# claudiok/clsim

Measured on AMD Instinct MI355X. Metric: propagated photons/sec (whole node), higher is better.
Workload: dtype f32

## Files before the change

### clsim_amd/_lib.py

```python
import ctypes as C
import os

HERE = os.path.dirname(os.path.abspath(__file__))
LIB_PATH = os.environ.get("CLSIMHIP_LIB", os.path.join(HERE, "libclsimhip.so"))

OK, ERR_ARGUMENT, ERR_STATE, ERR_CONFIG, ERR_DEVICE, ERR_IO = 0, -1, -2, -3, -4, -5
REFINDEX_ICECUBE, REFINDEX_TABLE, REFINDEX_DISPERSION = 0, 1, 2

DP = C.POINTER(C.c_double)


class Function(C.Structure):
    _fields_ = [("kind", C.c_int32), ("n", C.c_int32), ("start", C.c_double), ("step", C.c_double),
                ("values", DP), ("value", C.c_double), ("wavelengths", DP)]


class RandomValue(C.Structure):
    _fields_ = [("kind", C.c_int32), ("n", C.c_int32), ("first", C.c_double), ("spacing", C.c_double),
                ("y", DP), ("value", C.c_double), ("x", DP)]


class StepRequest(C.Structure):
    _fields_ = [("x", C.c_float), ("y", C.c_float), ("z", C.c_float), ("time", C.c_float),
                ("dx", C.c_float), ("dy", C.c_float), ("dz", C.c_float), ("length", C.c_float),
                ("pa", C.c_float), ("pb", C.c_float), ("kind", C.c_uint32), ("identifier", C.c_uint32),
                ("photons_per_step", C.c_uint32), ("num_photons_in_last_step", C.c_uint32), ("num_steps", C.c_uint64)]


class PPCConfig(C.Structure):
    _fields_ = [("photons_per_step", C.c_uint32), ("high_photons_per_step", C.c_uint32), ("use_high_photons_per_step_from", C.c_double),
                ("use_cascade_extension", C.c_int32), ("reserved", C.c_int32), ("medium_density", C.c_double), ("seed", C.c_uint64)]


class Distribution(C.Structure):
    _fields_ = [("kind", C.c_int32), ("value", C.c_float)]


class FlasherConfig(C.Structure):
    _fields_ = [("polar", Distribution), ("azimuthal", Distribution), ("time_delay", Distribution),
                ("interpret_in_polar_coordinates", C.c_int32), ("photons_per_step", C.c_uint32),
                ("max_bunch_size", C.c_uint32), ("bunch_size_granularity", C.c_uint32)]


class Axis(C.Structure):
    _fields_ = [("kind", C.c_int32), ("min", C.c_double), ("max", C.c_double), ("n_bins", C.c_uint32), ("power", C.c_uint32)]


class Polynomial(C.Structure):
    _fields_ = [("n", C.c_int32), ("coefficients", DP), ("range_min", C.c_double), ("range_max", C.c_double),
                ("underflow", C.c_double), ("overflow", C.c_double)]


class MediumDesc(C.Structure):
    _fields_ = [("num_layers", C.c_int32), ("layers_z_start", C.c_double), ("layers_height", C.c_double),
                ("min_wavelength", C.c_double), ("max_wavelength", C.c_double),
                ("lengths_kind", C.c_int32), ("abs_length", DP), ("sca_length", DP),
                ("alpha", C.c_double), ("kappa", C.c_double), ("A", C.c_double), ("B", C.c_double),
                ("D", C.c_double), ("E", C.c_double),
                ("a_dust400", DP), ("delta_tau", DP), ("b400", DP),
                ("n", C.c_double * 5), ("g", C.c_double * 5),
                ("scatter_kind", C.c_int32), ("liu_fraction", C.c_double), ("mean_cosine", C.c_double),
                ("has_anisotropy", C.c_int32), ("aniso_azimuth", C.c_double), ("aniso_k1", C.c_double),
                ("aniso_k2", C.c_double),
                ("has_pre_transform", C.c_int32), ("pre_renormalize", C.c_int32), ("pre_matrix", C.c_double * 9),
                ("has_post_transform", C.c_int32), ("post_renormalize", C.c_int32), ("post_matrix", C.c_double * 9),
                ("has_tilt", C.c_int32), ("tilt_num_distances", C.c_int32), ("tilt_num_z", C.c_int32),
                ("tilt_distances", DP), ("tilt_z_coordinates", DP), ("tilt_z_corrections", DP),
                ("tilt_azimuth", C.c_double),
                ("table_num_wavelengths", C.c_int32), ("table_start_wavelength", C.c_double),
                ("table_wavelength_step", C.c_double), ("table_store_as_16bit", C.c_int32),
                ("abs_length_table", DP), ("sca_length_table", DP),
                ("phase_index_kind", C.c_int32), ("group_index_kind", C.c_int32),
                ("phase_index_table", Function), ("group_index_table", Function)]


SYMBOLS = [
    "clsimhip_medium_create", "clsimhip_medium_create_from_ppc",
    "clsimhip_medium_create_from_photonics", "clsimhip_medium_describe", "clsimhip_medium_destroy",
    "clsimhip_icecube_dom_acceptance", "clsimhip_make_cherenkov_wlen_generator", "clsimhip_make_wlen_generator",
    "clsimhip_mwc_multipliers", "clsimhip_mwc_multipliers_from_file", "clsimhip_seed_streams",
    "clsimhip_create", "clsimhip_destroy", "clsimhip_last_error", "clsimhip_set_device", "clsimhip_get_device", "clsimhip_uses_pooled_kernel", "clsimhip_kernel_for_bunch",
    "clsimhip_step_series_blob_size", "clsimhip_encode_step_series", "clsimhip_decode_step_series",
    "clsimhip_photon_series_blob_size", "clsimhip_encode_photon_series", "clsimhip_decode_photon_series", "clsimhip_encode_portable_uint",
    "clsimhip_comm_get_unique_id", "clsimhip_comm_create", "clsimhip_comm_destroy", "clsimhip_gather_hits",
    "clsimhip_comm_info", "clsimhip_comm_statistics",
    "clsimhip_set_wlen_generators", "clsimhip_set_wlen_bias", "clsimhip_set_medium_properties", "clsimhip_set_geometry",
    "clsimhip_set_geometry_from_text_file",
    "clsimhip_set_enable_double_buffering", "clsimhip_set_double_precision", "clsimhip_set_stop_detected_photons",
    "clsimhip_set_save_all_photons", "clsimhip_set_save_all_photons_prescale",
    "clsimhip_set_fixed_number_of_absorption_lengths", "clsimhip_set_dom_pancake_factor",
    "clsimhip_set_photon_history_entries", "clsimhip_set_workgroup_size", "clsimhip_set_max_num_workitems",
    "clsimhip_compile", "clsimhip_get_max_workgroup_size", "clsimhip_initialize", "clsimhip_initialize_with_streams",
    "clsimhip_is_initialized", "clsimhip_enqueue_steps", "clsimhip_get_conversion_result", "clsimhip_get_result_histories",
    "clsimhip_release_result",
    "clsimhip_get_workgroup_size", "clsimhip_get_max_num_workitems", "clsimhip_queue_size",
    "clsimhip_more_photons_available", "clsimhip_get_statistics", "clsimhip_propagate_device",
    "clsimhip_set_concurrent_device_launches",
    "clsimhip_replace_indices_with_ids", "clsimhip_kernel_time_ms", "clsimhip_get_table", "clsimhip_get_rng_state",
    "clsimhip_eval_math", "clsimhip_check_math_exhaustive", "clsimhip_version",
    "clsimhip_eval_device_function", "clsimhip_eval_device_random", "clsimhip_get_option",
    "clsimhip_set_tuning", "clsimhip_get_tuning", "clsimhip_tabulator_set_tuning",
    "clsimhip_get_last_launch", "clsimhip_tabulator_get_last_launch",
    "clsimhip_count_generated_steps", "clsimhip_generate_steps_device", "clsimhip_generate_steps",
    "clsimhip_ppc_create", "clsimhip_ppc_destroy", "clsimhip_ppc_photons_per_meter", "clsimhip_ppc_enqueue", "clsimhip_shower_parameters",
    "clsimhip_flasher_correction_factor", "clsimhip_flasher_enqueue",
    "clsimhip_feeder_create", "clsimhip_feeder_destroy", "clsimhip_feeder_enqueue_light_source", "clsimhip_feeder_enqueue_steps",
    "clsimhip_feeder_enqueue_barrier", "clsimhip_feeder_barrier_active", "clsimhip_feeder_more_steps_available",
    "clsimhip_feeder_get_conversion_result", "clsimhip_feeder_release_result",
    "clsimhip_count_flasher_steps", "clsimhip_generate_flasher_steps_device", "clsimhip_generate_flasher_steps",
    "clsimhip_flasher_time_profile",
    "clsimhip_step_store_create", "clsimhip_step_store_destroy", "clsimhip_step_store_insert", "clsimhip_step_store_size",
    "clsimhip_step_store_count", "clsimhip_step_store_pop_bunch", "clsimhip_step_store_pop_bunch_filled",
    "clsimhip_step_store_size_with_dummy_fill",
    "clsimhip_tabulator_create", "clsimhip_tabulator_destroy", "clsimhip_tabulator_last_error",
    "clsimhip_tabulator_enqueue_steps", "clsimhip_tabulator_finish", "clsimhip_tabulator_get_shape",
    "clsimhip_tabulator_get_bin_content", "clsimhip_tabulator_get_bin_sums", "clsimhip_tabulator_get_bin_edges",
    "clsimhip_tabulator_get_statistics", "clsimhip_tabulator_get_rng_state", "clsimhip_tabulator_get_table",
    "clsimhip_tabulator_write_fits_file",
    "clsimhip_mcpe_generator_create", "clsimhip_mcpe_generator_destroy", "clsimhip_mcpe_generator_last_error",
    "clsimhip_mcpe_convert_host", "clsimhip_mcpe_convert_device", "clsimhip_set_mcpe_generator", "clsimhip_get_result_mcpes",
    "clsimhip_mcpe_series_host", "clsimhip_mcpe_series_workspace_bytes", "clsimhip_mcpe_series_device", "clsimhip_set_mcpe_series",
    "clsimhip_enqueue_steps_with_particles", "clsimhip_get_result_mcpe_series",
    "clsimhip_mcpe_merge_host", "clsimhip_mcpe_merge_workspace_bytes", "clsimhip_mcpe_merge_device", "clsimhip_set_mcpe_merging",
    "clsimhip_get_result_mcpe_merged",
    "clsimhip_pmt_generator_create", "clsimhip_pmt_generator_destroy", "clsimhip_pmt_generator_last_error",
    "clsimhip_pmt_convert_host", "clsimhip_pmt_convert_device", "clsimhip_set_pmt_generator", "clsimhip_get_result_pmt_hits",
]

KERNEL_FAMILIES = ("classic", "keep", "pool", "pool_keep", "tab4", "tab5")
LENGTHS_KINDS = ("constant", "icecube", "table")


def launched_dict(out):
    v = [int(x) for x in out]
    if v[0] < 0:
        return None
    return dict(family=KERNEL_FAMILIES[v[0]], lengths=LENGTHS_KINDS[v[1]], tilt=bool(v[2]), aniso=bool(v[3]), flasher=bool(v[4]), fast=bool(v[5]))


_lib = None


def load():
    global _lib
    if _lib is not None:
        return _lib
    if not os.path.exists(LIB_PATH):
        raise ImportError("%s is missing: run `python -c 'import __graft_entry__ as g; g.build()'` "
                          "(make -C clsim_amd/csrc); the HIP propagator has no fallback path" % LIB_PATH)
    try:
        import torch
    except ImportError:
        pass
    lib = C.CDLL(LIB_PATH)
    vp, sz, u32, u64, i32, dbl = C.c_void_p, C.c_size_t, C.c_uint32, C.c_uint64, C.c_int, C.c_double
    sig = {
        "clsimhip_medium_create": (i32, [C.POINTER(MediumDesc), C.POINTER(vp)]),
        "clsimhip_medium_create_from_ppc": (i32, [C.c_char_p, dbl, i32, C.POINTER(vp)]),
        "clsimhip_medium_create_from_photonics": (i32, [C.c_char_p, dbl, C.POINTER(vp)]),
        "clsimhip_medium_describe": (i32, [vp, C.POINTER(MediumDesc)]),
        "clsimhip_medium_destroy": (None, [vp]),
        "clsimhip_icecube_dom_acceptance": (i32, [dbl, dbl, DP, DP, DP]),
        "clsimhip_make_cherenkov_wlen_generator": (i32, [C.POINTER(Function), vp, DP, DP, DP]),
        "clsimhip_make_wlen_generator": (i32, [C.POINTER(Function), C.POINTER(Function), vp, C.POINTER(RandomValue), DP, DP, C.c_size_t]),
        "clsimhip_mwc_multipliers": (i32, [vp, sz]),
        "clsimhip_mwc_multipliers_from_file": (i32, [C.c_char_p, vp, sz]),
        "clsimhip_seed_streams": (i32, [vp, sz, u64, vp]),
        "clsimhip_create": (i32, [i32, C.POINTER(vp)]),
        "clsimhip_destroy": (None, [vp]),
        "clsimhip_last_error": (C.c_char_p, [vp]),
        "clsimhip_set_device": (i32, [vp, i32]),
        "clsimhip_get_device": (i32, [vp, C.POINTER(i32)]),
        "clsimhip_uses_pooled_kernel": (i32, [vp, C.POINTER(i32)]),
        "clsimhip_kernel_for_bunch": (i32, [vp, sz, C.POINTER(i32)]),
        "clsimhip_step_series_blob_size": (i32, [sz, C.POINTER(sz)]),
        "clsimhip_encode_step_series": (i32, [vp, sz, vp, sz, C.POINTER(sz)]),
        "clsimhip_decode_step_series": (i32, [vp, sz, vp, sz, C.POINTER(sz), C.POINTER(sz)]),
        "clsimhip_photon_series_blob_size": (i32, [sz, C.POINTER(sz)]),
        "clsimhip_encode_photon_series": (i32, [vp, sz, vp, sz, C.POINTER(sz)]),
        "clsimhip_decode_photon_series": (i32, [vp, sz, vp, sz, C.POINTER(sz), C.POINTER(sz)]),
        "clsimhip_encode_portable_uint": (i32, [u64, vp, C.POINTER(sz)]),
        "clsimhip_comm_get_unique_id": (i32, [vp]),
        "clsimhip_comm_create": (i32, [i32, i32, i32, vp, C.POINTER(vp)]),
        "clsimhip_comm_destroy": (None, [vp]),
        "clsimhip_comm_info": (i32, [vp, vp, vp, vp, vp, C.c_size_t]),
        "clsimhip_comm_statistics": (i32, [vp, vp, vp, vp, vp, i32]),
        "clsimhip_gather_hits": (i32, [vp, vp, vp, sz, i32, vp, sz, vp, vp]),
        "clsimhip_set_wlen_generators": (i32, [vp, C.POINTER(RandomValue), sz]),
        "clsimhip_set_wlen_bias": (i32, [vp, C.POINTER(Function)]),
        "clsimhip_set_medium_properties": (i32, [vp, vp]),
        "clsimhip_set_geometry": (i32, [vp, sz, vp, vp, vp, vp, vp, C.POINTER(C.c_char_p), dbl]),
        "clsimhip_set_geometry_from_text_file": (i32, [vp, C.c_char_p, dbl, C.c_int32, C.c_int32, u32, u32]),
        "clsimhip_set_enable_double_buffering": (i32, [vp, i32]),
        "clsimhip_set_double_precision": (i32, [vp, i32]),
        "clsimhip_set_stop_detected_photons": (i32, [vp, i32]),
        "clsimhip_set_save_all_photons": (i32, [vp, i32]),
        "clsimhip_set_save_all_photons_prescale": (i32, [vp, dbl]),
        "clsimhip_set_fixed_number_of_absorption_lengths": (i32, [vp, dbl]),
        "clsimhip_set_dom_pancake_factor": (i32, [vp, dbl]),
        "clsimhip_set_photon_history_entries": (i32, [vp, u32]),
        "clsimhip_set_workgroup_size": (i32, [vp, sz]),
        "clsimhip_set_max_num_workitems": (i32, [vp, sz]),
        "clsimhip_compile": (i32, [vp]),
        "clsimhip_get_max_workgroup_size": (i32, [vp, C.POINTER(sz)]),
        "clsimhip_initialize": (i32, [vp, u64]),
        "clsimhip_initialize_with_streams": (i32, [vp, vp, vp, sz]),
        "clsimhip_is_initialized": (i32, [vp]),
        "clsimhip_enqueue_steps": (i32, [vp, vp, sz, u32]),
        "clsimhip_get_conversion_result": (i32, [vp, C.POINTER(u32), C.POINTER(vp), C.POINTER(sz)]),
        "clsimhip_get_result_histories": (i32, [vp, vp, C.POINTER(C.POINTER(C.c_float)), C.POINTER(u32)]),
        "clsimhip_release_result": (i32, [vp, vp]),
        "clsimhip_get_workgroup_size": (i32, [vp, C.POINTER(sz)]),
        "clsimhip_get_max_num_workitems": (i32, [vp, C.POINTER(sz)]),
        "clsimhip_queue_size": (i32, [vp, C.POINTER(sz)]),
        "clsimhip_more_photons_available": (i32, [vp, C.POINTER(i32)]),
        "clsimhip_get_statistics": (i32, [vp, DP]),
        "clsimhip_propagate_device": (i32, [vp, vp, sz, sz, vp, sz, vp, vp]),
        "clsimhip_set_concurrent_device_launches": (i32, [vp, i32]),
        "clsimhip_replace_indices_with_ids": (i32, [vp, vp, sz]),
        "clsimhip_kernel_time_ms": (i32, [vp, i32, DP, C.POINTER(u64)]),
        "clsimhip_get_table": (C.c_long, [vp, C.c_char_p, DP, sz]),
        "clsimhip_get_rng_state": (i32, [vp, vp, sz]),
        "clsimhip_eval_math": (i32, [i32, i32, vp, vp, sz, vp]),
        "clsimhip_get_option": (i32, [vp, i32, DP]),
        "clsimhip_set_tuning": (i32, [vp, C.c_char_p, C.c_longlong]),
        "clsimhip_get_tuning": (i32, [vp, C.c_char_p, C.POINTER(C.c_longlong)]),
        "clsimhip_tabulator_set_tuning": (i32, [vp, C.c_char_p, C.c_longlong]),
        "clsimhip_get_last_launch": (i32, [vp, C.POINTER(C.c_int)]),
        "clsimhip_tabulator_get_last_launch": (i32, [vp, C.POINTER(C.c_int)]),
        "clsimhip_eval_device_function": (i32, [vp, i32, i32, i32, vp, sz, vp]),
        "clsimhip_eval_device_random": (i32, [vp, i32, i32, i32, vp, vp, sz, sz, vp]),
        "clsimhip_check_math_exhaustive": (i32, [i32, i32, i32, i32, vp, sz]),
        "clsimhip_version": (C.c_char_p, []),
        "clsimhip_ppc_create": (i32, [vp, C.POINTER(Function), C.POINTER(PPCConfig), C.POINTER(vp)]),
        "clsimhip_ppc_destroy": (None, [vp]),
        "clsimhip_ppc_photons_per_meter": (i32, [vp, i32, C.POINTER(C.c_double)]),
        "clsimhip_ppc_enqueue": (i32, [vp, vp, sz, C.POINTER(StepRequest), sz, C.POINTER(sz)]),
        "clsimhip_shower_parameters": (i32, [i32, C.c_double, C.c_double, C.POINTER(C.c_double)]),
        "clsimhip_flasher_correction_factor": (i32, [C.POINTER(Function), C.c_double, C.POINTER(Function), C.c_double, C.c_double, C.POINTER(C.c_double)]),
        "clsimhip_flasher_enqueue": (i32, [C.c_double, u64, vp, sz, vp, sz, C.POINTER(sz)]),
        "clsimhip_feeder_create": (i32, [vp, i32, u64, sz, sz, sz, C.POINTER(vp)]),
        "clsimhip_feeder_destroy": (None, [vp]),
        "clsimhip_feeder_enqueue_light_source": (i32, [vp, vp]),
        "clsimhip_feeder_enqueue_steps": (i32, [vp, u32, vp, sz]),
        "clsimhip_feeder_enqueue_barrier": (i32, [vp]),
        "clsimhip_feeder_barrier_active": (i32, [vp, C.POINTER(C.c_int)]),
        "clsimhip_feeder_more_steps_available": (i32, [vp, C.POINTER(C.c_int)]),
        "clsimhip_feeder_get_conversion_result": (i32, [vp, C.c_double, C.POINTER(C.c_int), C.POINTER(vp), C.POINTER(sz), C.POINTER(vp), C.POINTER(sz), C.POINTER(C.c_int)]),
        "clsimhip_feeder_release_result": (i32, [vp, vp]),
        "clsimhip_count_generated_steps": (i32, [C.POINTER(StepRequest), sz, sz, C.POINTER(sz), C.POINTER(sz)]),
        "clsimhip_generate_steps_device": (i32, [i32, C.POINTER(StepRequest), sz, u64, sz, vp, sz, vp, C.POINTER(sz)]),
        "clsimhip_generate_steps": (i32, [i32, C.POINTER(StepRequest), sz, u64, sz, vp, sz, C.POINTER(sz)]),
        "clsimhip_count_flasher_steps": (i32, [C.POINTER(FlasherConfig), vp, sz, C.POINTER(sz), C.POINTER(sz)]),
        "clsimhip_generate_flasher_steps_device": (i32, [i32, C.POINTER(FlasherConfig), vp, sz, u64, vp, sz, vp, C.POINTER(sz)]),
        "clsimhip_generate_flasher_steps": (i32, [i32, C.POINTER(FlasherConfig), vp, sz, u64, vp, sz, C.POINTER(sz)]),
        "clsimhip_flasher_time_profile": (i32, [dbl, vp, vp]),
        "clsimhip_step_store_create": (i32, [sz, C.POINTER(vp)]),
        "clsimhip_step_store_destroy": (None, [vp]),
        "clsimhip_step_store_insert": (i32, [vp, vp, sz]),
        "clsimhip_step_store_size": (i32, [vp, C.POINTER(sz)]),
        "clsimhip_step_store_count": (i32, [vp, u32, C.POINTER(u32)]),
        "clsimhip_step_store_pop_bunch": (i32, [vp, sz, vp, C.POINTER(sz)]),
        "clsimhip_step_store_pop_bunch_filled": (i32, [vp, sz, vp, vp]),
        "clsimhip_step_store_size_with_dummy_fill": (i32, [vp, sz, C.POINTER(sz)]),
        "clsimhip_tabulator_create": (i32, [i32, i32, C.POINTER(Axis), sz, i32, vp, C.POINTER(Function), C.POINTER(Polynomial),
                                            dbl, dbl, vp, vp, sz, C.POINTER(vp)]),
        "clsimhip_tabulator_destroy": (None, [vp]),
        "clsimhip_tabulator_last_error": (C.c_char_p, [vp]),
        "clsimhip_tabulator_enqueue_steps": (i32, [vp, vp, sz, DP]),
        "clsimhip_tabulator_finish": (i32, [vp]),
        "clsimhip_tabulator_get_shape": (i32, [vp, C.POINTER(sz), C.POINTER(sz), C.POINTER(sz)]),
        "clsimhip_tabulator_get_bin_content": (i32, [vp, vp, sz, i32, i32]),
        "clsimhip_tabulator_get_bin_sums": (i32, [vp, vp, sz, i32]),
        "clsimhip_tabulator_get_bin_edges": (i32, [vp, i32, DP, sz]),
        "clsimhip_tabulator_get_statistics": (i32, [vp, DP]),
        "clsimhip_tabulator_get_rng_state": (i32, [vp, vp, sz]),
        "clsimhip_tabulator_get_table": (C.c_long, [vp, C.c_char_p, DP, sz]),
        "clsimhip_mcpe_generator_create": (i32, [C.POINTER(Function), sz, sz, vp, vp, vp, C.POINTER(Polynomial), dbl, dbl, dbl, u64, C.POINTER(vp)]),
        "clsimhip_mcpe_generator_destroy": (None, [vp]),
        "clsimhip_mcpe_generator_last_error": (C.c_char_p, [vp]),
        "clsimhip_mcpe_convert_host": (i32, [vp, vp, sz, vp, sz, C.POINTER(sz), vp]),
        "clsimhip_mcpe_convert_device": (i32, [vp, i32, vp, vp, sz, vp, sz, vp, vp]),
        "clsimhip_set_mcpe_generator": (i32, [vp, vp, i32]),
        "clsimhip_get_result_mcpes": (i32, [vp, vp, C.POINTER(vp), C.POINTER(sz)]),
        "clsimhip_mcpe_series_host": (i32, [vp, vp, sz, vp, sz, vp, sz, vp, vp, C.POINTER(sz), C.POINTER(sz), vp]),
        "clsimhip_mcpe_series_workspace_bytes": (sz, [sz, sz, sz]),
        "clsimhip_mcpe_series_device": (i32, [vp, i32, vp, vp, sz, vp, sz, vp, sz, vp, vp, vp, vp, sz, vp]),
        "clsimhip_set_mcpe_series": (i32, [vp, i32]),
        "clsimhip_enqueue_steps_with_particles": (i32, [vp, vp, sz, u32, vp, sz, vp, sz]),
        "clsimhip_get_result_mcpe_series": (i32, [vp, vp, C.POINTER(vp), C.POINTER(sz), C.POINTER(vp), C.POINTER(sz), C.POINTER(u64)]),
        "clsimhip_mcpe_merge_host": (i32, [vp, sz, vp, sz, C.c_double, vp, vp, vp, vp, C.POINTER(sz), C.POINTER(sz)]),
        "clsimhip_mcpe_merge_workspace_bytes": (sz, [sz]),
        "clsimhip_mcpe_merge_device": (i32, [vp, i32, vp, vp, vp, sz, C.c_double, vp, vp, vp, vp, vp, vp, sz, vp]),
        "clsimhip_set_mcpe_merging": (i32, [vp, i32, C.c_double]),
        "clsimhip_get_result_mcpe_merged": (i32, [vp, vp, C.POINTER(vp), C.POINTER(sz), C.POINTER(vp), C.POINTER(sz), C.POINTER(vp), C.POINTER(sz), C.POINTER(vp)]),
        "clsimhip_pmt_generator_create": (i32, [C.POINTER(Function), sz, vp, sz, vp, sz, vp, sz, u64, C.POINTER(vp)]),
        "clsimhip_pmt_generator_destroy": (None, [vp]),
        "clsimhip_pmt_generator_last_error": (C.c_char_p, [vp]),
        "clsimhip_pmt_convert_host": (i32, [vp, vp, sz, vp, sz, C.POINTER(sz), vp]),
        "clsimhip_pmt_convert_device": (i32, [vp, i32, vp, vp, sz, vp, sz, vp, vp]),
        "clsimhip_set_pmt_generator": (i32, [vp, vp, i32]),
        "clsimhip_get_result_pmt_hits": (i32, [vp, vp, C.POINTER(vp), C.POINTER(sz)]),
        "clsimhip_tabulator_write_fits_file": (i32, [vp, C.c_char_p, C.POINTER(C.c_char_p), C.POINTER(C.c_int32), C.POINTER(C.c_int64), C.POINTER(C.c_double), sz]),
    }
    for name in SYMBOLS:
        fn = getattr(lib, name)
        fn.restype, fn.argtypes = sig[name]
    _lib = lib
    return lib
```

### clsim_amd/converter.py

```python
import ctypes as C
import math
import os

import numpy as np

from . import _lib
from .synthetic import PHOTON_DTYPE, STEP_DTYPE

NANOMETER = 1e-9


class I3CLSimStepToPhotonConverter_exception(RuntimeError):

    def __init__(self, msg, code=0):
        RuntimeError.__init__(self, msg)
        self.code = code


def _check(rc, handle=None):
    if rc != _lib.OK:
        msg = _lib.load().clsimhip_last_error(handle)
        raise I3CLSimStepToPhotonConverter_exception((msg or b"").decode() or ("status %d" % rc), rc)


# ... 650 lines not shown
    def MorePhotonsAvailable(self):
        v = C.c_int()
        self._call("clsimhip_more_photons_available", C.byref(v))
        return bool(v.value)

    def GetStatistics(self):
        out = (C.c_double * 8)()
        self._call("clsimhip_get_statistics", out)
        keys = ["TotalDeviceTime", "TotalHostTime", "NumKernelCalls", "TotalNumPhotonsGenerated",
                "TotalNumPhotonsAtDOMs", "AverageDeviceTimePerPhoton", "AverageHostTimePerPhoton", "DeviceUtilization"]
        return dict(zip(keys, list(out)))

    def GetTotalDeviceTime(self): return self.GetStatistics()["TotalDeviceTime"]
    def GetTotalHostTime(self): return self.GetStatistics()["TotalHostTime"]
    def GetNumKernelCalls(self): return int(self.GetStatistics()["NumKernelCalls"])
    def GetTotalNumPhotonsGenerated(self): return int(self.GetStatistics()["TotalNumPhotonsGenerated"])
    def GetTotalNumPhotonsAtDOMs(self): return int(self.GetStatistics()["TotalNumPhotonsAtDOMs"])

    _KERNELS = {"auto": 0, "pool": 1, "classic": 2}

    def SetTuning(self, key, value):
        if key == "kernel" and isinstance(value, str):
            value = self._KERNELS[value]
        self._call("clsimhip_set_tuning", key.encode(), int(value))

    def GetTuning(self, key):
        v = C.c_longlong()
        self._call("clsimhip_get_tuning", key.encode(), C.byref(v))
        return v.value

    def _option(self, which):
        v = C.c_double()
        self._call("clsimhip_get_option", int(which), C.byref(v))
        return v.value

    def GetEnableDoubleBuffering(self): return self._option(0) != 0.0
    def GetDoublePrecision(self): return self._option(1) != 0.0
    def GetStopDetectedPhotons(self): return self._option(2) != 0.0
    def GetSaveAllPhotons(self): return self._option(3) != 0.0
    def GetSaveAllPhotonsPrescale(self): return self._option(4)
    def GetFixedNumberOfAbsorptionLengths(self): return self._option(5)
    def GetDOMPancakeFactor(self): return self._option(6)
    def GetPhotonHistoryEntries(self): return int(self._option(7))

    def PropagateDevice(self, d_steps, n, d_photons, capacity, d_hit_count, stream=0, rng_offset=0):
        self._call("clsimhip_propagate_device", C.c_void_p(d_steps), int(n), int(rng_offset), C.c_void_p(d_photons),
                   int(capacity), C.c_void_p(d_hit_count), C.c_void_p(stream))

    def SetConcurrentDeviceLaunches(self, k):
        self._call("clsimhip_set_concurrent_device_launches", int(k))

    def ReplaceIndicesWithIDs(self, photons):
        photons = np.ascontiguousarray(photons, dtype=PHOTON_DTYPE)
        self._call("clsimhip_replace_indices_with_ids", photons.ctypes.data_as(C.c_void_p), len(photons))
        return photons

    def KernelTimeMs(self, reset=False):
        total, launches = C.c_double(), C.c_uint64()
        self._call("clsimhip_kernel_time_ms", int(bool(reset)), C.byref(total), C.byref(launches))
        return total.value, launches.value

    def GetTable(self, name):
        n = self._lib.clsimhip_get_table(self._h, name.encode(), None, 0)
        if n < 0:
            _check(int(n), self._h)
        out = np.zeros(n, dtype=np.float64)
        self._lib.clsimhip_get_table(self._h, name.encode(), _dp(out), n)
        return out

    def KernelForBunch(self, n_steps):
        v = C.c_int32()
        self._call("clsimhip_kernel_for_bunch", int(n_steps), C.byref(v))
        return "pool" if v.value else "classic"

    def UsesPooledKernel(self):
        v = C.c_int32()
        self._call("clsimhip_uses_pooled_kernel", C.byref(v))
        return bool(v.value)

    def GetLastLaunch(self):
        out = (C.c_int * 6)()
        self._call("clsimhip_get_last_launch", out)
        return _lib.launched_dict(out)

    EVAL = {"lengths": 0, "refraction": 1, "wavelength_bias": 2, "tilt": 3, "abs_len_scaling": 4, "pre_scatter_transform": 5,
            "post_scatter_transform": 6}
    EVAL_RANDOM = {"uniform": 0, "wavelength": 1, "scattering_cosine": 2}

    def EvaluateOnDevice(self, what, values, layer=0, fast=False):
        v = np.asarray(values, dtype=np.float32)
        inp = np.zeros((len(v), 4), dtype=np.float32)
        if v.ndim == 1:
            inp[:, 0] = v
        else:
            inp[:, :v.shape[1]] = v
        out = np.zeros_like(inp)
        self._call("clsimhip_eval_device_function", self.EVAL[what], int(layer), int(bool(fast)), inp.ctypes.data_as(C.c_void_p), len(inp),
                   out.ctypes.data_as(C.c_void_p))
        return out

    def SampleOnDevice(self, what, x, a, draws, generator=0, fast=False):
        xs = np.ascontiguousarray(x, dtype=np.uint64).copy()
        a32 = np.ascontiguousarray(a, dtype=np.uint32)
        out = np.zeros((len(xs), int(draws)), dtype=np.float32)
        self._call("clsimhip_eval_device_random", self.EVAL_RANDOM[what], int(generator), int(bool(fast)), xs.ctypes.data_as(C.c_void_p),
                   a32.ctypes.data_as(C.c_void_p), len(xs), int(draws), out.ctypes.data_as(C.c_void_p))
        return out, xs

    def GetRNGState(self, count):
        x = np.zeros(count, dtype=np.uint64)
        self._call("clsimhip_get_rng_state", x.ctypes.data_as(C.c_void_p), count)
        return x


def initializeHIP(device, geometry, medium, wavelengthGenerationBias, wavelengthGenerators,
                  enableDoubleBuffering=False, doublePrecision=False, stopDetectedPhotons=True, saveAllPhotons=False,
                  saveAllPhotonsPrescale=0.01, fixedNumberOfAbsorptionLengths=float("nan"), pancakeFactor=1.0,
                  photonHistoryEntries=0, limitWorkgroupSize=0, approximateNumberOfWorkItems=262144,
                  seed=12345, streams=None, tuning=None, mcpeGenerator=None, keepPhotons=True, mcpeSeries=False, pmtHitGenerator=None, mcpeMergeWindow=None):
    conv = I3CLSimStepToPhotonConverterHIP(device)
    for key, value in (tuning or {}).items():
        conv.SetTuning(key, value)
    conv.SetWlenGenerators(wavelengthGenerators)
    conv.SetWlenBias(wavelengthGenerationBias)
    conv.SetMediumProperties(medium)
    conv.SetGeometry(geometry)
    conv.SetEnableDoubleBuffering(enableDoubleBuffering)
    conv.SetDoublePrecision(doublePrecision)
    conv.SetStopDetectedPhotons(stopDetectedPhotons)
    conv.SetSaveAllPhotons(saveAllPhotons)
    conv.SetSaveAllPhotonsPrescale(saveAllPhotonsPrescale)
    conv.SetFixedNumberOfAbsorptionLengths(fixedNumberOfAbsorptionLengths)
    conv.SetDOMPancakeFactor(pancakeFactor)
    conv.SetPhotonHistoryEntries(photonHistoryEntries)
    if mcpeGenerator is not None:
        conv.SetMCPEGenerator(mcpeGenerator, keepPhotons)
    if mcpeSeries:
        conv.SetMCPESeries(True)
    if mcpeMergeWindow is not None:
        conv.SetMCPEMerging(mcpeMergeWindow)
    if pmtHitGenerator is not None:
        conv.SetPMTHitGenerator(pmtHitGenerator, keepPhotons)
    conv.Compile()
    max_wg = conv.GetMaxWorkgroupSize()
    if limitWorkgroupSize:
        max_wg = min(limitWorkgroupSize, max_wg)
    conv.SetWorkgroupSize(max_wg)
    wg = max_wg
    max_items = (int(approximateNumberOfWorkItems) // wg) * wg
    if max_items == 0:
        max_items = wg
    conv.SetMaxNumWorkitems(max_items)
    if streams is not None:
        conv.InitializeWithStreams(streams[0][:max_items], streams[1][:max_items])
    else:
        conv.Initialize(seed)
    return conv


REQUEST_DTYPE = np.dtype([("x", "<f4"), ("y", "<f4"), ("z", "<f4"), ("time", "<f4"), ("dx", "<f4"), ("dy", "<f4"), ("dz", "<f4"),
                          ("length", "<f4"), ("pa", "<f4"), ("pb", "<f4"), ("kind", "<u4"), ("identifier", "<u4"),
                          ("photons_per_step", "<u4"), ("num_photons_in_last_step", "<u4"), ("num_steps", "<u8")])
STEPS_CASCADE, STEPS_MUON_CASCADE, STEPS_MUON = 0, 1, 2


def CountGeneratedSteps(requests, granularity=1):
# ... 184 lines not shown
```

### clsim_amd/csrc/c_api.cpp

```cpp
#include <cstring>
#include <map>
#include <memory>
#include <mutex>

#include "converter.h"
#include "lightsource.h"
#include "feeder.h"
#include "tabulator.h"
#include "step_store.h"
#include "flasher.h"
#include "mcpe.h"
#include "mcpe_merge.h"
#include "pmt_hits.h"

using namespace clsimhip;

struct clsimhip_converter { Converter impl; explicit clsimhip_converter(int dev) : impl(dev) {} };
struct clsimhip_medium { MediumData data; };
struct clsimhip_mcpe_generator { std::shared_ptr<McpeGenerator> impl; };
struct clsimhip_pmt_generator { std::shared_ptr<PmtHitGenerator> impl; };
struct clsimhip_tabulator {
    std::unique_ptr<Tabulator> impl;
};

// ... 304 lines not shown
        need(path, "path"); need(a_out, "a_out");
        if (!load_multipliers_from_file(path, a_out, count)) throw Error(CLSIMHIP_ERR_IO, std::string("could not read ") + std::to_string(count) + " multipliers from " + path);
    });
}
int clsimhip_seed_streams(const uint32_t *a, size_t count, uint64_t seed, uint64_t *x_out)
{
    return guarded(nullptr, [&] { need(a, "a"); need(x_out, "x_out"); seed_streams(a, count, seed, x_out); });
}

int clsimhip_create(int device_ordinal, clsimhip_converter **out)
{
    return guarded(nullptr, [&] { need(out, "out"); *out = new clsimhip_converter(device_ordinal); });
}
void clsimhip_destroy(clsimhip_converter *c) { delete c; }
int clsimhip_set_device(clsimhip_converter *c, int device_ordinal)
{
    return guarded(c, [&] { need(c, "converter"); c->impl.set_device(device_ordinal); });
}
int clsimhip_set_concurrent_device_launches(clsimhip_converter *c, int k)
{
    return guarded(c, [&] { need(c, "converter"); c->impl.set_concurrent_device_launches(k); });
}
int clsimhip_step_series_blob_size(size_t n, size_t *bytes)
{
    return guarded(nullptr, [&] { need(bytes, "bytes"); *bytes = series_blob_size(n, sizeof(clsimhip_step)); });
}
int clsimhip_encode_step_series(const clsimhip_step *steps, size_t n, uint8_t *out, size_t capacity, size_t *written)
{
    return guarded(nullptr, [&] { series_encode(steps, n, sizeof(clsimhip_step), 0u, out, capacity, written); });
}
int clsimhip_decode_step_series(const uint8_t *blob, size_t bytes, clsimhip_step *steps_out, size_t capacity, size_t *n, size_t *consumed)
{
    return guarded(nullptr, [&] { series_decode(blob, bytes, sizeof(clsimhip_step), 0u, "I3CLSimStep", steps_out, capacity, n, consumed); });
}
int clsimhip_photon_series_blob_size(size_t n, size_t *bytes)
{
    return guarded(nullptr, [&] { need(bytes, "bytes"); *bytes = series_blob_size(n, sizeof(clsimhip_photon)); });
}
int clsimhip_encode_photon_series(const clsimhip_photon *photons, size_t n, uint8_t *out, size_t capacity, size_t *written)
{
    return guarded(nullptr, [&] { series_encode(photons, n, sizeof(clsimhip_photon), 0u, out, capacity, written); });
}
int clsimhip_decode_photon_series(const uint8_t *blob, size_t bytes, clsimhip_photon *photons_out, size_t capacity, size_t *n, size_t *consumed)
{
    return guarded(nullptr, [&] { series_decode(blob, bytes, sizeof(clsimhip_photon), 0u, "I3CLSimPhoton", photons_out, capacity, n, consumed); });
}
int clsimhip_encode_portable_uint(uint64_t value, uint8_t out[9], size_t *written)
{
    return guarded(nullptr, [&] { need(out, "out"); need(written, "written"); *written = portable_uint_encode(value, out); });
}
int clsimhip_comm_get_unique_id(uint8_t id[CLSIMHIP_UNIQUE_ID_BYTES])
{
    return guarded(nullptr, [&] { need(id, "id"); comm_unique_id(id); });
}
int clsimhip_comm_create(int device_ordinal, int rank, int world_size, const uint8_t id[CLSIMHIP_UNIQUE_ID_BYTES], clsimhip_comm **out)
{
    return guarded(nullptr, [&] { need(out, "out"); *out = reinterpret_cast<clsimhip_comm *>(comm_create(device_ordinal, rank, world_size, id)); });
}
void clsimhip_comm_destroy(clsimhip_comm *comm) { comm_destroy(reinterpret_cast<Comm *>(comm)); }
int clsimhip_comm_info(clsimhip_comm *comm, int *rccl_ranks, int *rccl_rank, int *device_ordinal, char *pci_bus_id, size_t pci_bus_id_bytes)
{
    return guarded(nullptr, [&] { comm_info(reinterpret_cast<Comm *>(comm), rccl_ranks, rccl_rank, device_ordinal, pci_bus_id, pci_bus_id_bytes); });
}
int clsimhip_comm_statistics(clsimhip_comm *comm, uint64_t *gathers, double *gather_ms, uint64_t *records_sent, uint64_t *records_received, int reset)
{
    return guarded(nullptr, [&] { comm_statistics(reinterpret_cast<Comm *>(comm), gathers, gather_ms, records_sent, records_received, reset != 0); });
}
int clsimhip_gather_hits(clsimhip_comm *comm, const void *d_photons, const void *d_hit_count, size_t capacity, int root,
                         void *d_gathered, size_t gathered_capacity, uint64_t *counts_out, void *hip_stream)
{
    return guarded(nullptr, [&] {
        comm_gather_hits(reinterpret_cast<Comm *>(comm), d_photons, d_hit_count, capacity, root, d_gathered, gathered_capacity, counts_out,
                         static_cast<hipStream_t>(hip_stream));
    });
}
int clsimhip_uses_pooled_kernel(const clsimhip_converter *c, int *out)
{
    return guarded_const(c, [&] { need(c, "converter"); need(out, "out"); *out = c->impl.uses_pooled_kernel() ? 1 : 0; });
}
int clsimhip_kernel_for_bunch(const clsimhip_converter *c, size_t n_steps, int *out)
{
    return guarded_const(c, [&] { need(c, "converter"); need(out, "out"); *out = c->impl.pooled_for(n_steps) ? 1 : 0; });
}
int clsimhip_get_device(const clsimhip_converter *c, int *out)
{
    return guarded_const(c, [&] { need(c, "converter"); need(out, "out"); *out = c->impl.device(); });
}

int clsimhip_set_wlen_generators(clsimhip_converter *c, const clsimhip_random_value *gens, size_t n)
{
    return guarded(c, [&] {
        need(c, "converter"); need(gens, "generators");
        std::vector<RandomValueData> v(n);
        for (size_t i = 0; i < n; ++i) {
            v[i].kind = gens[i].kind;
            if (gens[i].kind == CLSIMHIP_RANDOM_INTERPOLATED) {
                if (gens[i].n < 2 || !gens[i].y) throw Error(CLSIMHIP_ERR_ARGUMENT, "At least two entries have to be specified in the vector passed to I3CLSimRandomValueInterpolatedDistribution().");
                v[i].first = gens[i].first; v[i].spacing = gens[i].spacing;
                v[i].y.assign(gens[i].y, gens[i].y + gens[i].n);
            } else if (gens[i].kind == CLSIMHIP_RANDOM_INTERPOLATED_X) {
                if (gens[i].n < 2 || !gens[i].y || !gens[i].x) throw Error(CLSIMHIP_ERR_ARGUMENT, "At least two entries have to be specified in the vectors passed to I3CLSimRandomValueInterpolatedDistribution().");
                v[i].x.assign(gens[i].x, gens[i].x + gens[i].n);
                v[i].y.assign(gens[i].y, gens[i].y + gens[i].n);
            } else if (gens[i].kind == CLSIMHIP_RANDOM_CONSTANT) {
                v[i].value = gens[i].value;
            } else if (gens[i].kind == CLSIMHIP_RANDOM_CHERENKOV_NO_DISPERSION) {
                v[i].first = gens[i].first; v[i].spacing = gens[i].spacing;
            } else
                throw Error(CLSIMHIP_ERR_ARGUMENT, "unknown random value kind");
        }
        c->impl.set_wlen_generators(std::move(v));
    });
}
int clsimhip_set_wlen_bias(clsimhip_converter *c, const clsimhip_function *bias)
{
    return guarded(c, [&] { need(c, "converter"); c->impl.set_wlen_bias(function_from(bias)); });
}
int clsimhip_set_medium_properties(clsimhip_converter *c, const clsimhip_medium *m)
{
    return guarded(c, [&] { need(c, "converter"); need(m, "medium"); c->impl.set_medium(m->data); });
}
int clsimhip_set_geometry(clsimhip_converter *c, size_t n, const int32_t *string_ids, const uint32_t *dom_ids, const double *x,
                          const double *y, const double *z, const char *const *subdetectors, double om_radius)
{
    return guarded(c, [&] {
        need(c, "converter"); need(string_ids, "string_ids"); need(dom_ids, "dom_ids"); need(x, "x"); need(y, "y"); need(z, "z");
        need(subdetectors, "subdetectors");
        GeometryInput g;
        g.string_ids.assign(string_ids, string_ids + n); g.dom_ids.assign(dom_ids, dom_ids + n);
        g.x.assign(x, x + n); g.y.assign(y, y + n); g.z.assign(z, z + n);
        g.subdetectors.resize(n);
        for (size_t i = 0; i < n; ++i) { need(subdetectors[i], "subdetector name"); g.subdetectors[i] = subdetectors[i]; }
        g.om_radius = om_radius;
        c->impl.set_geometry(std::move(g));
    });
}
int clsimhip_set_geometry_from_text_file(clsimhip_converter *c, const char *filename, double om_radius, int32_t string_id_min,
                                         int32_t string_id_max, uint32_t dom_id_min, uint32_t dom_id_max)
{
    return guarded(c, [&] {
        need(c, "converter"); need(filename, "filename");
        c->impl.set_geometry(geometry_from_text_file(filename, om_radius, string_id_min, string_id_max, dom_id_min, dom_id_max));
    });
}
#define SETTER(name, type, call) \
    int name(clsimhip_converter *c, type value) { return guarded(c, [&] { need(c, "converter"); c->impl.call; }); }
SETTER(clsimhip_set_enable_double_buffering, int, set_double_buffering(value != 0))
SETTER(clsimhip_set_double_precision, int, set_double_precision(value != 0))
SETTER(clsimhip_set_stop_detected_photons, int, set_stop_detected(value != 0))
SETTER(clsimhip_set_save_all_photons, int, set_save_all(value != 0))
SETTER(clsimhip_set_save_all_photons_prescale, double, set_save_all_prescale(value))
SETTER(clsimhip_set_fixed_number_of_absorption_lengths, double, set_fixed_abs_lengths(value))
SETTER(clsimhip_set_dom_pancake_factor, double, set_pancake(value))
SETTER(clsimhip_set_photon_history_entries, uint32_t, set_history_entries(value))
SETTER(clsimhip_set_workgroup_size, size_t, set_workgroup_size(value))
SETTER(clsimhip_set_max_num_workitems, size_t, set_max_num_workitems(value))
#undef SETTER

int clsimhip_compile(clsimhip_converter *c) { return guarded(c, [&] { need(c, "converter"); c->impl.compile(); }); }
int clsimhip_get_max_workgroup_size(const clsimhip_converter *c, size_t *out)
{
    return guarded_const(c, [&] { need(c, "converter"); need(out, "out"); *out = c->impl.max_workgroup_size(); });
}
int clsimhip_initialize(clsimhip_converter *c, uint64_t seed) { return guarded(c, [&] { need(c, "converter"); c->impl.initialize(seed); }); }
int clsimhip_initialize_with_streams(clsimhip_converter *c, const uint64_t *x, const uint32_t *a, size_t count)
{
// ... 587 lines not shown
```

### clsim_amd/csrc/converter.cpp

```cpp
#include "converter.h"
#include "mcpe.h"
#include "mcpe_merge.h"
#include "pmt_hits.h"

#include <chrono>
#include <cmath>
#include <cstdio>
#include <cstring>
#include <fstream>

namespace clsimhip {
[[maybe_unused]] constexpr size_t kCensusBytes = 4u << 20;


static_assert(sizeof(clsimhip_step) == sizeof(DevStep), "step layouts");
static_assert(sizeof(clsimhip_photon) == sizeof(DevPhoton), "photon layouts");
constexpr uint32_t kQueueSlots = 256;
constexpr size_t kPooledKernelMinSteps = 524288;

hipError_t Converter::launch(const KParams &P, const LaunchTuning &tuning, hipStream_t stream) const
{
    KVariant v = tables_.variant;
    const bool pooled = tuning.pooled_for(P.n_steps, concurrent_launches_);
    v.grid = tuning.grid;
    v.generic_only = tuning.generic_only;
    KLaunched launched;
    v.launched = &launched;
    const hipError_t err = v.keep_detected ? (pooled ? launch_pool_keep_kernel(P, v, stream) : launch_keep_kernel(P, v, stream))
                                           : (pooled ? launch_pool_kernel(P, v, stream) : launch_prop_kernel(P, v, stream));
    if (launched.family >= 0) {
        std::lock_guard<std::mutex> lk(launched_mutex_);
        launched_ = launched;
    }
    return err;
}

void Converter::apply_kernel_choice()
{
    LaunchTuning &t = tuning_;
    t.derived = true;
    t.use_pool = pool_possible_ && t.kernel != 2;
    t.pool_min_steps = (t.kernel != 0) ? 0 : kPooledKernelMinSteps;
    if (t.tuned_pool_min_steps >= 0) t.pool_min_steps = static_cast<size_t>(t.tuned_pool_min_steps);
    t.pool_max_steps = pool_kernel_max_steps();
    if (t.tuned_pool_max_steps >= 0) t.pool_max_steps = std::min(t.pool_max_steps, static_cast<size_t>(t.tuned_pool_max_steps));
}

namespace {
struct TuningKey {
    const char *name;
    long long lo, hi;
    bool shapes_tables;
    long long (*get)(const LaunchTuning &, const TableTuning &);
    void (*set)(LaunchTuning &, TableTuning &, long long);
};
#define LAUNCH_FIELD(f) false, [](const LaunchTuning &l, const TableTuning &) { return static_cast<long long>(l.f); }, \
                        [](LaunchTuning &l, TableTuning &, long long v) { l.f = static_cast<decltype(l.f)>(v); }
#define TABLE_FIELD(f) true, [](const LaunchTuning &, const TableTuning &t) { return static_cast<long long>(t.f); }, \
                       [](LaunchTuning &, TableTuning &t, long long v) { t.f = static_cast<decltype(t.f)>(v); }
const TuningKey kTuningKeys[] = {
    {"kernel", 0, 2, LAUNCH_FIELD(kernel)},
    {"pool_min_steps", -1, 1ll << 40, false,
     [](const LaunchTuning &l, const TableTuning &) { return l.derived ? static_cast<long long>(l.pool_min_steps) : l.tuned_pool_min_steps; },
     [](LaunchTuning &l, TableTuning &, long long v) { l.tuned_pool_min_steps = v; }},
    {"pool_max_steps", -1, 1ll << 40, false,
     [](const LaunchTuning &l, const TableTuning &) { return l.derived ? static_cast<long long>(l.pool_max_steps) : l.tuned_pool_max_steps; },
     [](LaunchTuning &l, TableTuning &, long long v) { l.tuned_pool_max_steps = v; }},
    {"pool_ring", 0, 4096, LAUNCH_FIELD(pool_ring)},
    {"k_new", 0, 4096, LAUNCH_FIELD(k_new)},
    {"k_search", 0, 64, LAUNCH_FIELD(k_search)},
    {"slices", 0, 65535, LAUNCH_FIELD(slices)},
    {"k_pop", 0, 64, LAUNCH_FIELD(k_pop)},
    {"k_wait", -1, 255, LAUNCH_FIELD(k_wait)},
    {"k_aim", -1, 64, LAUNCH_FIELD(k_aim)},
    {"grid", 0, 1 << 20, LAUNCH_FIELD(grid)},
    {"generic_kernels", 0, 1, LAUNCH_FIELD(generic_only)},
    {"result_min_records", 1, 1ll << 32, LAUNCH_FIELD(result_min_records)},
    {"string_map_cells", 8, 4096, TABLE_FIELD(string_map_cells)},
    {"dom_map_cells", 4, 512, TABLE_FIELD(dom_map_cells)},
    {"named_search", 0, 1, TABLE_FIELD(named_search)},
};
#undef LAUNCH_FIELD
#undef TABLE_FIELD

const TuningKey &tuning_key(const std::string &key)
{
    for (const TuningKey &t : kTuningKeys) if (key == t.name) return t;
    throw Error(CLSIMHIP_ERR_ARGUMENT, "no tuning key named " + key);
}
}

void Converter::set_tuning(const std::string &key, long long value)
{
    const TuningKey &k = tuning_key(key);
    if (value < k.lo || value > k.hi)
        throw Error(CLSIMHIP_ERR_ARGUMENT, "tuning " + key + ": " + std::to_string(value) + " is outside " + std::to_string(k.lo) + " ... " + std::to_string(k.hi));
    if (k.shapes_tables && compiled_) throw Error(CLSIMHIP_ERR_STATE, "tuning " + key + " shapes a table of Compile(): set it before Compile()");
    std::lock_guard<std::mutex> lk(tuning_mutex_);
    k.set(tuning_, table_tuning_, value);
    if (initialized_) apply_kernel_choice();
}

long long Converter::get_tuning(const std::string &key) const
{
    const TuningKey &k = tuning_key(key);
    std::lock_guard<std::mutex> lk(tuning_mutex_);
    return k.get(tuning_, table_tuning_);
}

void Converter::set_concurrent_device_launches(int k)
{
    if (k < 1 || k > 16) throw Error(CLSIMHIP_ERR_ARGUMENT, "concurrent device launches: 1 ... 16");
    concurrent_launches_ = k;
}

Converter::Converter(int device) : device_(device)
{
    if (device < 0) throw Error(CLSIMHIP_ERR_ARGUMENT, "device ordinal out of range");
}

Converter::~Converter()
{
    if (in_queue_) in_queue_->close();
    if (out_queue_) out_queue_->close();
    if (worker_.joinable()) worker_.join();
    in_queue_.reset();
    release_device();
}

void Converter::release_device()
{
    if (!dev_.stream) return;
    DeviceGuard on_device(device_, std::nothrow);
    handed_out_.clear();
    if (out_queue_) {
        Result r;
        while (out_queue_->get_for(r, 0)) {}
    }
    dev_ = DeviceState();
    step_pool_.reset();
    result_pool_.reset();
    mcpe_pool_.reset();
    series_pool_.reset();
    merge_pool_.reset();
    pmt_pool_.reset();
    bunch_pool_.reset();
}

void Converter::set_device(int device)
{
    guard();
    if (device < 0) throw Error(CLSIMHIP_ERR_ARGUMENT, "device ordinal out of range");
    device_ = device;
}

void Converter::check_worker() const
{
    std::lock_guard<std::mutex> lk(fatal_mutex_);
    if (worker_failed_) throw Error(CLSIMHIP_ERR_DEVICE, "the converter's worker thread stopped after a device error: " + fatal_error_);
}

void Converter::set_wlen_generators(std::vector<RandomValueData> g)
{
    guard();
    for (const RandomValueData &r : g) {
        if (r.kind == CLSIMHIP_RANDOM_CONSTANT) {
            if (!std::isfinite(r.value) || !(r.value > 0.)) throw Error(CLSIMHIP_ERR_ARGUMENT, "a constant wavelength must be finite and positive");
        } else if (r.kind == CLSIMHIP_RANDOM_CHERENKOV_NO_DISPERSION) {
            if (std::isnan(r.first)) throw Error(CLSIMHIP_ERR_ARGUMENT, "The \"fromWlen\" argument must not be NaN!");
            if (std::isnan(r.spacing)) throw Error(CLSIMHIP_ERR_ARGUMENT, "The \"toWlen\" argument must not be NaN!");
            if (r.first > r.spacing) throw Error(CLSIMHIP_ERR_ARGUMENT, "The \"fromWlen\" argument must not be greater than \"toWlen\".");
            if (!(r.first > 0.) || !std::isfinite(r.spacing)) throw Error(CLSIMHIP_ERR_ARGUMENT, "the wavelength range must be positive and finite");
        } else {
            if (r.kind == CLSIMHIP_RANDOM_INTERPOLATED_X) {
                if (r.x.size() != r.y.size()) throw Error(CLSIMHIP_ERR_ARGUMENT, "The \"x\" and \"y\" vectors must have the same size!");
                for (size_t i = 0; i < r.x.size(); ++i)
                    if (!std::isfinite(r.x[i]) || !(r.x[i] > 0.) || (i > 0 && !(r.x[i] > r.x[i - 1])))
                        throw Error(CLSIMHIP_ERR_ARGUMENT, "the wavelengths of a distribution must be positive, finite and ascending");
            } else if (!std::isfinite(r.first) || !(r.first > 0.) || !std::isfinite(r.spacing) || !(r.spacing > 0.))
                throw Error(CLSIMHIP_ERR_ARGUMENT, "a wavelength distribution needs a positive first wavelength and spacing");
            double sum = 0.;
            for (double y : r.y) {
                if (!std::isfinite(y) || y < 0.) throw Error(CLSIMHIP_ERR_ARGUMENT, "wavelength distribution values must be finite and non-negative");
                sum += y;
            }
            if (!(sum > 0.)) throw Error(CLSIMHIP_ERR_ARGUMENT, "a wavelength distribution must not be zero everywhere");
        }
    }
    compiled_ = false;
    generators_ = std::move(g);
// ... 976 lines not shown
```

### clsim_amd/csrc/converter.h

```cpp
#pragma once
#include <hip/hip_runtime.h>

#include <atomic>
#include <chrono>
#include <condition_variable>
#include <cstdio>
#include <deque>
#include <memory>
#include <mutex>
#include <thread>

#include "hip_resources.h"
#include "host_model.h"
#include "kparams.h"
#include "prop_launch.h"

namespace clsimhip {

class McpeGenerator;
class PmtHitGenerator;
struct alignas(16) SeriesParticle16 { uint8_t bytes[16]; };

struct Comm;
void comm_unique_id(uint8_t id[CLSIMHIP_UNIQUE_ID_BYTES]);
Comm *comm_create(int device, int rank, int world, const uint8_t id[CLSIMHIP_UNIQUE_ID_BYTES]);
void comm_destroy(Comm *c);
void comm_info(Comm *c, int *ranks, int *rank, int *device, char *pci_bus_id, size_t pci_bytes);
void comm_statistics(Comm *c, uint64_t *gathers, double *gather_ms, uint64_t *records_sent, uint64_t *records_received, bool reset);
void comm_gather_hits(Comm *c, const void *d_photons, const void *d_hit_count, size_t capacity, int root, void *d_gathered,
                      size_t gathered_capacity, uint64_t *counts_out, hipStream_t stream);

struct CompiledTables {
    KParams params{};
    KVariant variant{};
    std::vector<uint32_t> lds_image;
    std::vector<float> len_table;
    std::vector<uint32_t> prox_map;
    std::vector<uint32_t> dom_prox;
    std::vector<float> dom_centres;
    std::vector<uint32_t> dom_named;
    GeoTables geo;
    std::map<std::string, std::vector<double>> named;
};
struct TableTuning {
    int string_map_cells = 512;
    int dom_map_cells = 256;
    bool named_search = true;
};
CompiledTables compile_tables(const MediumData &medium, const GeometryInput &geometry,
                              const std::vector<RandomValueData> &generators, const FunctionData &bias,
                              double pancake_factor, const TableTuning &tuning = TableTuning());

template <class T>
class BoundedQueue {
public:
    explicit BoundedQueue(size_t cap) : cap_(cap) {}
    void put(T v)
    {
        std::unique_lock<std::mutex> lk(m_);
        cond_.wait(lk, [&] { return q_.size() < cap_ + waiting_ || closed_; });
        if (closed_) return;
        q_.push_back(std::move(v));
        cond_.notify_all();
    }
    bool get(T &out)
    {
        std::unique_lock<std::mutex> lk(m_);
        ++waiting_;
        cond_.notify_all();
        cond_.wait(lk, [&] { return !q_.empty() || closed_; });
        --waiting_;
        if (q_.empty()) return false;
        out = std::move(q_.front());
        q_.pop_front();
        cond_.notify_all();
        return true;
    }
    bool get_for(T &out, long us)
    {
        std::unique_lock<std::mutex> lk(m_);
        ++waiting_;
        cond_.notify_all();
        const bool got = cond_.wait_for(lk, std::chrono::microseconds(us), [&] { return !q_.empty() || closed_; });
        --waiting_;
        if (!got || q_.empty()) { cond_.notify_all(); return false; }
        out = std::move(q_.front());
        q_.pop_front();
        cond_.notify_all();
        return true;
    }
    bool closed() const { std::lock_guard<std::mutex> lk(m_); return closed_; }
    size_t size() const { std::lock_guard<std::mutex> lk(m_); return q_.size(); }
    bool empty() const { return size() == 0; }
    void close() { std::lock_guard<std::mutex> lk(m_); closed_ = true; cond_.notify_all(); }
private:
    size_t cap_;
// ... 37 lines not shown

    explicit PinnedPool(const PinnedPoolPolicy &policy) : policy_(policy) {}
    Lease take(size_t records, size_t new_capacity, int device)
    {
        const size_t bytes = new_capacity * sizeof(T);
        PinnedBuffer<T> retired;
        {
            std::lock_guard<std::mutex> lk(mutex_);
            size_t best = free_.size(), smallest = free_.size();
            for (size_t i = 0; i < free_.size(); ++i) {
                const size_t c = free_[i].capacity;
                if (c >= records && (best == free_.size() || c < free_[best].capacity)) best = i;
                if (smallest == free_.size() || c < free_[smallest].capacity) smallest = i;
            }
            if (best != free_.size()) {
                Lease found(this, std::move(free_[best].buf), free_[best].capacity);
                free_.erase(free_.begin() + static_cast<std::ptrdiff_t>(best));
                return found;
            }
            if (refused_) return Lease();
            if (made_ >= policy_.max_buffers || (bytes_ + bytes > policy_.max_bytes && made_ >= 3)) {
                if (free_.empty()) {
                    if (policy_.all_out_notice && !noticed_) {
                        noticed_ = true;
                        std::fprintf(stderr, policy_.all_out_notice, made_, records);
                    }
                    return Lease();
                }
                const size_t gone = free_[smallest].capacity * sizeof(T);
                if (bytes_ - gone + bytes > policy_.max_bytes && made_ - 1 >= 3) return Lease();
                retired = std::move(free_[smallest].buf);
                free_.erase(free_.begin() + static_cast<std::ptrdiff_t>(smallest));
                bytes_ -= gone;
                --made_;
            }
            ++made_;
            bytes_ += bytes;
        }
        DeviceGuard on_device(device);
        retired.reset();
        PinnedBuffer<T> fresh;
        if (!fresh.try_alloc(new_capacity)) {
            std::lock_guard<std::mutex> lk(mutex_);
            --made_;
            bytes_ -= bytes;
            refused_ = true;
            return Lease();
        }
        return Lease(this, std::move(fresh), new_capacity);
    }
    void reset()
    {
        std::lock_guard<std::mutex> lk(mutex_);
        free_.clear();
        made_ = 0; bytes_ = 0; refused_ = false; noticed_ = false;
    }

private:
    void give(PinnedBuffer<T> buf, size_t capacity)
    {
        std::lock_guard<std::mutex> lk(mutex_);
        free_.push_back(Entry{std::move(buf), capacity});
    }
    struct Entry { PinnedBuffer<T> buf; size_t capacity; };
    const PinnedPoolPolicy policy_;
    std::mutex mutex_;
    std::vector<Entry> free_;
    int made_ = 0;
    size_t bytes_ = 0;
    bool refused_ = false;
    bool noticed_ = false;
};

struct LaunchTuning {
    int kernel = 0;
    long long tuned_pool_min_steps = -1;
    long long tuned_pool_max_steps = -1;
    int pool_ring = 0, k_pop = 0;
    int k_new = 0, slices = 0;
    int k_search = 0;
    int k_wait = -1, k_aim = -1;
    int grid = 0;
    bool generic_only = false;
    size_t result_min_records = 65536;
    bool derived = false;
    bool use_pool = false;
    size_t pool_min_steps = 0;
    size_t pool_max_steps = 0;
    bool pooled_for(size_t n_steps, int concurrent_launches) const
    {
        return use_pool && n_steps <= pool_max_steps && n_steps * static_cast<size_t>(concurrent_launches) >= pool_min_steps;
    }
};

class Converter {
public:
    explicit Converter(int device);
    ~Converter();

    void set_wlen_generators(std::vector<RandomValueData> g);
    void set_wlen_bias(FunctionData b);
    void set_medium(MediumData m);
    void set_geometry(GeometryInput g);
    void set_double_buffering(bool v) { guard(); double_buffering_ = v; }
    void set_double_precision(bool v) { guard(); double_precision_ = v; }
    void set_stop_detected(bool v) { guard(); stop_detected_ = v; }
    void set_save_all(bool v) { guard(); save_all_ = v; }
    void set_save_all_prescale(double v) { guard(); save_all_prescale_ = v; }
    void set_fixed_abs_lengths(double v) { guard(); fixed_abs_lengths_ = v; }
    void set_pancake(double v) { guard(); pancake_ = v; }
    void set_history_entries(uint32_t v) { guard(); history_entries_ = v; }
    void set_workgroup_size(size_t v);
    void set_max_num_workitems(size_t v);
    void set_mcpe_generator(std::shared_ptr<McpeGenerator> g, bool keep_photons);
    void set_mcpe_series(bool on) { guard(); compiled_ = false; series_ = on; }
    void set_mcpe_merging(bool on, double window);
    void set_pmt_generator(std::shared_ptr<PmtHitGenerator> g, bool keep_photons);

    void compile();
    void initialize(uint64_t seed);
    void initialize_with_streams(const uint64_t *x, const uint32_t *a, size_t count);
    bool initialized() const { return initialized_; }
    size_t max_workgroup_size() const { return static_cast<size_t>(prop_kernel_block_size()); }
    size_t workgroup_size() const { return workgroup_size_; }
    size_t max_num_workitems() const { return max_workitems_; }

    void enqueue_steps(const clsimhip_step *steps, size_t n, uint32_t identifier);
    void enqueue_steps(const clsimhip_step *steps, size_t n, uint32_t identifier, const clsimhip_mcpe_particle *particles, size_t n_particles,
                       const clsimhip_mcpe_mask *masked, size_t n_masked);
    void get_result(uint32_t *identifier, const clsimhip_photon **photons, size_t *n);
    void result_histories(const clsimhip_photon *photons, const float **histories, uint32_t *entries);
    void result_mcpes(const clsimhip_photon *photons, const clsimhip_mcpe **mcpes, size_t *n);
    void result_mcpe_series(const clsimhip_photon *photons, const clsimhip_mcpe **mcpes, size_t *n, const clsimhip_mcpe_series **series, size_t *n_series,
                            uint64_t *n_masked);
    void result_mcpe_merged(const clsimhip_photon *photons, const clsimhip_mcpe_merged **merged, size_t *n_merged, const clsimhip_mcpe_series **series,
                            size_t *n_series, const clsimhip_mcpe_parent **parents, size_t *n_parents, const clsimhip_mcpe_parent_range **ranges);
    void result_pmt_hits(const clsimhip_photon *photons, const clsimhip_pmt_hit **hits, size_t *n);
    void release_result(const clsimhip_photon *photons);
    size_t queue_size() const;
    bool more_photons_available() const;
    void statistics(double out[8]) const;
    double option(int which) const;

    void propagate_device(const void *d_steps, size_t n, size_t rng_offset, void *d_photons, size_t capacity,
                          void *d_hit_count, hipStream_t stream);
    void replace_indices(clsimhip_photon *photons, size_t n) const;
    void kernel_time(bool reset, double *total_ms, uint64_t *launches);
    long get_table(const std::string &name, double *out, size_t cap) const;
    void get_rng_state(uint64_t *x, size_t count);
    void eval_device_function(int what, int layer, bool fast, const float *in4, size_t n, float *out4);
    void eval_device_random(int what, int generator, bool fast, uint64_t *x, const uint32_t *a, size_t n_streams, size_t draws, float *out);
    void debug_counters(uint32_t out[4]);
    void set_device(int device);
    int device() const { return device_; }
    bool pooled_for(size_t n_steps) const { need_init(); return tuning_snapshot().pooled_for(n_steps, concurrent_launches_); }
    void set_tuning(const std::string &key, long long value);
    long long get_tuning(const std::string &key) const;
    void set_concurrent_device_launches(int k);
    int concurrent_device_launches() const { return concurrent_launches_; }
    bool uses_pooled_kernel() const { need_init(); const LaunchTuning t = tuning_snapshot(); return t.use_pool && t.pool_min_steps == 0; }
    KLaunched last_launch() const { std::lock_guard<std::mutex> lk(launched_mutex_); return launched_; }

private:
    using StepPool = PinnedPool<clsimhip_step>;
    using PhotonPool = PinnedPool<clsimhip_photon>;
    using McpePool = PinnedPool<clsimhip_mcpe>;
    using SeriesPool = PinnedPool<clsimhip_mcpe_series>;
    using PmtHitPool = PinnedPool<clsimhip_pmt_hit>;
    using BlobPool = PinnedPool<uint8_t>;
    struct Job {
        uint32_t id = 0; size_t n = 0; uint64_t generated = 0; StepPool::Lease pinned; std::vector<clsimhip_step> steps;
        SeriesBunch bunch; BlobPool::Lease bunch_pinned; std::vector<SeriesParticle16> bunch_blob;
    };
    struct Result {
        uint32_t id = 0;
        PhotonPool::Lease pinned;
        size_t count = 0;
        std::unique_ptr<std::vector<clsimhip_photon>> photons;
        std::unique_ptr<std::vector<float>> histories;
        const clsimhip_photon *data() const { return pinned ? pinned.get() : (photons ? photons->data() : nullptr); }
        McpePool::Lease mcpe_pinned;
        size_t mcpe_count = 0;
        std::unique_ptr<std::vector<clsimhip_mcpe>> mcpes;
        std::unique_ptr<clsimhip_photon> handle;
        const clsimhip_mcpe *mcpe_data() const { return mcpe_pinned ? mcpe_pinned.get() : (mcpes ? mcpes->data() : nullptr); }
        SeriesPool::Lease series_pinned;
        size_t series_count = 0;
        uint64_t masked = 0;
        std::unique_ptr<std::vector<clsimhip_mcpe_series>> series;
        const clsimhip_mcpe_series *series_data() const { return series_pinned ? series_pinned.get() : (series ? series->data() : nullptr); }
        BlobPool::Lease merge_pinned;
        std::unique_ptr<std::vector<uint64_t>> merge_blob;
        size_t merged_count = 0, parent_count = 0;
        const uint8_t *merge_data() const { return merge_pinned ? merge_pinned.get() : (merge_blob ? reinterpret_cast<const uint8_t *>(merge_blob->data()) : nullptr); }
        PmtHitPool::Lease pmt_pinned;
        size_t pmt_count = 0;
        std::unique_ptr<std::vector<clsimhip_pmt_hit>> pmt_hits;
        const clsimhip_pmt_hit *pmt_data() const { return pmt_pinned ? pmt_pinned.get() : (pmt_hits ? pmt_hits->data() : nullptr); }
    };

    void guard() const { if (initialized_) throw Error(CLSIMHIP_ERR_STATE, "I3CLSimStepToPhotonConverterHIP already initialized!"); }
    void need_init() const { if (!initialized_) throw Error(CLSIMHIP_ERR_STATE, "I3CLSimStepToPhotonConverterHIP is not initialized!"); }
    struct DeviceState;
    void setup_device_buffers(DeviceState &D);
    void release_device();
    void worker();
    void check_worker() const;
    KParams launch_params(const LaunchTuning &tuning, const void *d_steps, size_t n, size_t rng_offset, void *d_photons, size_t capacity, void *d_hits,
                          hipStream_t stream);

    int device_;
    std::vector<RandomValueData> generators_;
    FunctionData bias_;
    MediumData medium_;
    GeometryInput geometry_;
    bool have_bias_ = false, have_medium_ = false, have_geometry_ = false;
    bool double_buffering_ = false, double_precision_ = false, stop_detected_ = false, save_all_ = false;
    double save_all_prescale_ = 0.001, fixed_abs_lengths_ = NAN, pancake_ = 1.0;
    uint32_t history_entries_ = 0;
    size_t workgroup_size_ = 0, max_workitems_ = 0;
    uint32_t max_output_photons_ = 0;

    std::shared_ptr<McpeGenerator> mcpe_;
    bool keep_photons_ = true;
    bool series_ = false;
    bool merging_ = false;
    double merge_window_ = 0.;
    std::shared_ptr<PmtHitGenerator> pmt_;
    bool pmt_keep_photons_ = true;
    bool carries_photons() const { return !(mcpe_ && !keep_photons_) && !(pmt_ && !pmt_keep_photons_); }

    std::atomic<bool> compiled_{false}, initialized_{false};
    CompiledTables tables_;

    PhotonPool result_pool_{PinnedPoolPolicy{6, SIZE_MAX, nullptr}};
    McpePool mcpe_pool_{PinnedPoolPolicy{6, SIZE_MAX, nullptr}};
    SeriesPool series_pool_{PinnedPoolPolicy{6, SIZE_MAX, nullptr}};
    BlobPool merge_pool_{PinnedPoolPolicy{6, SIZE_MAX, nullptr}};
    PmtHitPool pmt_pool_{PinnedPoolPolicy{6, SIZE_MAX, nullptr}};
    BlobPool bunch_pool_{PinnedPoolPolicy{8, size_t{1} << 28, nullptr}};
    size_t result_capacity(size_t records, size_t min_records) const;
    StepPool step_pool_{PinnedPoolPolicy{8, size_t{1} << 30,
        "clsimhip: all %d page-locked step buffers are in flight; this bunch of %zu steps is staged through pageable memory\n"}};

    struct Slot {
        Event start, stop, counted, uploaded;
        DeviceBuffer<DevStep> d_steps;
        DeviceBuffer<DevPhoton> d_photons;
        DeviceBuffer<uint32_t> d_hit_count;
        DeviceBuffer<float> d_hist_out;
        PinnedBuffer<float> h_hist;
        PinnedBuffer<clsimhip_step> h_steps;
        StepPool::Lease step_lease;
        PinnedBuffer<uint32_t> h_hit_count;
        DeviceBuffer<clsimhip_mcpe> d_mcpes;
        DeviceBuffer<uint32_t> d_mcpe_counters;
        PinnedBuffer<uint32_t> h_mcpe_counters;
        DeviceBuffer<clsimhip_pmt_hit> d_pmt_hits;
        DeviceBuffer<uint32_t> d_pmt_counters;
        PinnedBuffer<uint32_t> h_pmt_counters;
        DeviceBuffer<uint8_t> d_series_workspace;
        size_t series_workspace_bytes = 0;
        DeviceBuffer<clsimhip_mcpe> d_sorted;
        DeviceBuffer<clsimhip_mcpe_series> d_series;
        DeviceBuffer<uint32_t> d_series_counts;
        PinnedBuffer<uint32_t> h_series_counts;
        DeviceBuffer<uint8_t> d_merge_workspace;
        size_t merge_workspace_bytes = 0;
        DeviceBuffer<clsimhip_mcpe_merged> d_merged;
        DeviceBuffer<clsimhip_mcpe_series> d_merged_series;
        DeviceBuffer<clsimhip_mcpe_parent> d_parents;
        DeviceBuffer<clsimhip_mcpe_parent_range> d_ranges;
        DeviceBuffer<uint32_t> d_merge_counts;
        PinnedBuffer<uint32_t> h_merge_counts;
        BlobPool::Lease bunch_lease;
        PinnedBuffer<uint8_t> h_bunch;
        size_t h_bunch_bytes = 0;
        uint32_t id = 0;
        uint64_t generated = 0;
        size_t result_min_records = 0;
    };
    struct DeviceState {
        std::vector<std::pair<Event, Event>> pending_events, free_events;
        Stream stream;
        Stream copy_stream;
        Stream upload_stream;
        Slot slots[2];
        DeviceBuffer<uint32_t> tables;
        DeviceBuffer<int16_t> dom_tx, dom_ty;
        DeviceBuffer<float> dom_tz;
        DeviceBuffer<float> len_table;
        DeviceBuffer<uint32_t> prox_map, dom_prox, dom_named;
        DeviceBuffer<float> dom_centres;
        DeviceBuffer<float> hist_ring;
        DeviceBuffer<uint64_t> rng_x;
        DeviceBuffer<uint32_t> rng_a;
        DeviceBuffer<int16_t> id_strings;
        DeviceBuffer<uint16_t> id_doms;
        DeviceBuffer<uint32_t> id_dom_start;
        DeviceBuffer<WorkRecord> work;
        DeviceBuffer<uint32_t> queue;
        uint32_t *last_queue = nullptr;
#ifdef CLSIMHIP_CENSUS
        DeviceBuffer<unsigned long long> census;
#endif
    };
    DeviceState dev_;
    int num_slots_ = 1;
    void submit(Slot &s, Job &job);
    void finish(Slot &s, std::chrono::steady_clock::time_point &last_done, bool &first);
    uint32_t queue_slot_ = 0;
    int concurrent_launches_ = 1;
    LaunchTuning tuning_;
    TableTuning table_tuning_;
    bool pool_possible_ = false;
    void apply_kernel_choice();
    mutable std::mutex tuning_mutex_;
    LaunchTuning tuning_snapshot() const { std::lock_guard<std::mutex> lk(tuning_mutex_); return tuning_; }
    hipError_t launch(const KParams &P, const LaunchTuning &tuning, hipStream_t stream) const;
    mutable std::mutex launched_mutex_;
    mutable KLaunched launched_;

    std::unique_ptr<BoundedQueue<Job>> in_queue_;
    std::unique_ptr<BoundedQueue<Result>> out_queue_;
    std::thread worker_;
    mutable std::mutex fatal_mutex_;
    std::string fatal_error_;
    bool worker_failed_ = false;
    mutable std::mutex results_mutex_;
    std::map<const clsimhip_photon *, Result> handed_out_;

    mutable std::mutex stats_mutex_;
    uint64_t total_device_ns_ = 0, total_host_ns_ = 0, num_kernel_calls_ = 0, photons_generated_ = 0, photons_at_doms_ = 0;

    std::mutex ev_mutex_;
    double dev_total_ms_ = 0;
    uint64_t dev_launches_ = 0;
};

}
```

### clsim_amd/csrc/detmath.hip.h

```cpp
#pragma once
#include <hip/hip_runtime.h>
#include <stdint.h>

#include "math_tables.h"

#define DM __device__ __forceinline__

namespace dm {

DM float fma_(float a, float b, float c) { return __builtin_fmaf(a, b, c); }
DM float sqrt_(float a) { return __builtin_sqrtf(a); }
DM float rsqrt_(float a) { return 1.0f / __builtin_sqrtf(a); }
DM float rint_(float a) { return __builtin_rintf(a); }

DM uint32_t f2u(float f) { return __builtin_bit_cast(uint32_t, f); }
DM float u2f(uint32_t u) { return __builtin_bit_cast(float, u); }

DM float rcp_(float x)
{
    const float r0 = __builtin_amdgcn_rcpf(x);
    const float e0 = fma_(-x, r0, 1.0f);
    return fma_(e0, r0, r0);
}
DM float rcp_of_rcp_(float b, float x)
{
    const float e = fma_(-b, x, 1.0f);
    return fma_(e, x, x);
}
DM bool div_near_ok_(float a) { return __builtin_fabsf(a) >= 9.094947017729282e-13f; }
DM float div_near_with_(float a, float b, float y)
{
    const float q0 = a * y;
    const float r0 = fma_(-b, q0, a);
    const float q1 = fma_(r0, y, q0);
    const float r1 = fma_(-b, q1, a);
    return fma_(r1, y, q1);
}
DM float div_near_(float a, float b) { return div_near_with_(a, b, rcp_(b)); }
DM float sqrt_near_(float x)
{
    const float s = __builtin_amdgcn_sqrtf(x);
    const uint32_t dn = __builtin_elementwise_sub_sat(f2u(s), 1u);
    const float s_dn = u2f(dn), s_up = u2f(f2u(s) + 1u);
    const float r_dn = fma_(-s_dn, s, x);
    const float r_up = fma_(-s_up, s, x);
    uint32_t m_dn, m_up;
    asm("v_med3_i32 %0, %1, 0, 1" : "=v"(m_dn) : "v"(r_dn));
    asm("v_med3_i32 %0, %1, 0, 1" : "=v"(m_up) : "v"(r_up));
    return u2f(dn + m_dn + m_up);
}
DM float rsqrt_near_(float x) { return rcp_(sqrt_near_(x)); }
DM bool rsqrt_unit_ok_(float x) { return (f2u(x) - (0x3f800000u - 1023u)) <= 2046u; }
DM float rsqrt_unit_(float x)
{
    const int d = (int)(f2u(x) - 0x3f800000u);
    const uint32_t above = 0x3f800000u - ((uint32_t)d & ~1u);
    const uint32_t below = 0x3f800000u + ((uint32_t)(3 - d) >> 2);
    return u2f((d < 0) ? below : above);
}

constexpr uint32_t kMathLogWords = 4u * MT_LOG_ROWS, kMathScWords = 2u * MT_SC_ROWS, kMathTableWords = (kMathLogWords + kMathScWords + 3u) & ~3u;
static __device__ const float kLogTable[kMathLogWords] = MT_LOG_TABLE;
static __device__ const float kScTable[kMathScWords] = MT_SC_TABLE;
static const float kLogTableHost[kMathLogWords] = MT_LOG_TABLE;
static const float kScTableHost[kMathScWords] = MT_SC_TABLE;

constexpr float LN2_HI = 0.693359375f;
constexpr float LN2_LO = -2.12194440e-4f;
constexpr float LOG2E = 1.44269504088896341f;

DM float log_poly(float r)
{
    float p = 7.0376836292e-2f;
    p = fma_(p, r, -1.1514610310e-1f);
    p = fma_(p, r, 1.1676998740e-1f);
    p = fma_(p, r, -1.2420140846e-1f);
    p = fma_(p, r, 1.4249322787e-1f);
    p = fma_(p, r, -1.6668057665e-1f);
    p = fma_(p, r, 2.0000714765e-1f);
    p = fma_(p, r, -2.4999993993e-1f);
    p = fma_(p, r, 3.3333331174e-1f);
    return p;
}

DM float frexp_sqrt2(float x, int &e)
// ... 232 lines not shown
```

### clsim_amd/csrc/kparams.h

```cpp
#pragma once
#include <stdint.h>

namespace clsimhip {

constexpr int kMaxGenerators = 8;
constexpr int kMaxSubdetectors = 9;

#pragma pack(push, 1)
struct DevStep {
    float x, y, z, t;
    float theta, phi, length, beta;
    uint32_t num_photons;
    float weight;
    uint32_t identifier;
    uint32_t source_type_and_pad;
};
struct DevPhoton {
    uint32_t w[20];
};
#pragma pack(pop)
constexpr int kSubQueues = 8;
constexpr int kQueueHeadStride = 32;
constexpr int kQueueWords = 512;

struct WorkRecord {
    DevStep step;
    uint64_t x;
    uint32_t a;
    uint32_t done;
};
static_assert(sizeof(WorkRecord) == 64, "work record");
static_assert(sizeof(DevStep) == 48, "step record");
static_assert(sizeof(DevPhoton) == 80, "photon record");

struct KParams {
    const uint32_t *tables;
    uint32_t table_words;
    const DevStep *steps;
    uint32_t n_steps;
    uint64_t *rng_x;
    const uint32_t *rng_a;
    DevPhoton *out;
    uint32_t *hit_count;
    uint32_t max_hits;
    uint32_t *queue;
    int32_t k_new;
    int32_t k_search;
    int32_t k_wait;
    int32_t k_aim;
    int32_t slices;
    int32_t pool_ready, k_pop;
    int32_t chip_share;
#ifdef CLSIMHIP_CENSUS
    unsigned long long *census;
#endif
    WorkRecord *work;
    const float *len_table;
    float *hist_ring;
    float *hist_out;
    int32_t history_n;
    int32_t has_fixed_abs;
    float fixed_abs;
    const uint32_t *prox_map;
    int32_t prox_n;
    float prox_x0, prox_y0, prox_inv_cell, prox_reach;
    const uint4 *dom_cells;
    const float4 *dom_centres;
    const uint4 *dom_named;
    const int16_t *id_strings;
    const uint16_t *id_doms;
    const uint32_t *id_dom_start;
    int32_t dprox_nx, dprox_ny, dprox_nz;
    float dprox_x0, dprox_y0, dprox_z0, dprox_inv_cell;
    float dprox_radius;
    const int16_t *dom_tx;
    const int16_t *dom_ty;
    const float *dom_tz;
    int32_t dom_in_lds;
    uint32_t off_dom_xy, off_dom_z;

    int32_t num_layers;
    float layer_bottom, layer_thickness, recip_thickness;
    uint32_t off_layers;
    float neg_kappa, abs_A, neg_B, neg_alpha, ref_wlen_recip, nanometer;
    float n[5], g[5], micrometer, c_light;
    int32_t len_tab_n;
    float len_tab_start, len_tab_step;
    int32_t phase_kind, group_kind;
    int32_t phase_n, group_n;
    float phase_start, phase_step, group_start, group_step;
    uint32_t off_phase, off_group;
    float mix_frac, mix_frac_rest, liu_beta, hg_g, hg_one_minus_g2, hg_one_plus_g2, hg_two_g;
    float an_l[3], an_rl[3], an_azx, an_azy, an_mazy, an_B2, abs_corr_const;
    float pre[9], post[9];
    int32_t has_abs_corr, has_pre, has_post, pre_renorm, post_renorm;
    int32_t scatter_kind;
    float tilt_const;
    int32_t tilt_nd, tilt_nz;
    float tilt_first_z, tilt_dz, tilt_lnx, tilt_lny;
    uint32_t off_tilt_dist, off_tilt_zcorr;
    uint32_t off_tilt_bins;
    float tilt_inner_dist[6];

    float rcp_tilt_dz, rcp_layer_thickness, rcp_mix_frac, rcp_mix_frac_rest, rcp_hg_two_g;
    uint32_t div_ok;

    int32_t num_gen;
    int32_t gen_kind[kMaxGenerators], gen_n[kMaxGenerators];
    float gen_first[kMaxGenerators], gen_spacing[kMaxGenerators], gen_value[kMaxGenerators];
    uint32_t off_gen_yv[kMaxGenerators], off_gen_ycum[kMaxGenerators];
    uint32_t off_gen_xv[kMaxGenerators];
    int32_t bias_kind, bias_n;
    float bias_start, bias_step, bias_value;
    uint32_t off_bias;

    double *tab_bins;
    double *tab_sq_bins;
    float tab_ref[12];
    uint32_t off_tab;
    int32_t tab_axes_kind, tab_full_azimuth;
    int32_t tab_ndim;
    float tab_scale[5], tab_offset[5];
    int32_t tab_inverse[5], tab_nbins[5];
    float tab_inv_exp[5];
    uint32_t tab_stride[5];
    uint32_t tab_tiled, tab_tile_stride[3];
    uint32_t tab_tile_bits[3];
    uint32_t tab_std;
    float tab_max0, tab_max3, tab_min_inv_groupvel, tab_tan_thetac, tab_volume_step;
    int32_t ang_n;
    uint32_t off_ang;
    int32_t ang_has_min, ang_has_max;
    float ang_min, ang_max, ang_underflow, ang_overflow;

    int32_t has_pancake;
    float pancake, unpancake;
    float om_radius, om_radius_sq, string_max_radius_sq, string_max_radius;
    int32_t num_strings, num_sets, max_layers, num_subdet;
    uint32_t off_strings;
    uint32_t off_sets;
    uint32_t off_layer_to_om;
    uint32_t off_subdet;
    float dom_mul_x, dom_mul_y;
    uint32_t k_packed;
};

struct KLaunched {
    int family = -1, lengths = -1, tilt = -1, aniso = -1, flasher = -1, fast = -1;
};

struct KVariant {
    int lengths;
    bool tilt;
    bool aniso;
    bool flasher;
    bool tabulate = false;
    bool keep_detected = false;
    bool fast = false;
    int grid = 0;
    bool generic_only = false;
    bool tab_fast = false;
    KLaunched *launched = nullptr;
};

}
```

### clsim_amd/csrc/prop_device.hip.h

```cpp
#pragma once
#include <hip/hip_runtime.h>

#include "detmath.hip.h"
#include "../../include/clsimhip.h"
#include "kparams.h"
#include "instrument.hip.h"

namespace clsimhip {

#ifndef CLSIMHIP_BLOCK
#define CLSIMHIP_BLOCK 256
#define CLSIMHIP_MIN_WAVES 7
#endif
constexpr int kBlock = CLSIMHIP_BLOCK;
constexpr int kMinWavesPerSimd = CLSIMHIP_MIN_WAVES;
constexpr int kWavesPerBlock = kBlock / 64;
constexpr int kStageRecords = 8;
constexpr int kStubWords = 16;
#ifndef CLSIMHIP_PRIO_SHIFT
#define CLSIMHIP_PRIO_SHIFT 1
#endif
constexpr int kPrioShift = CLSIMHIP_PRIO_SHIFT;
constexpr int kTabSlots = 512;
#ifndef CLSIMHIP_TAB_POOL
#define CLSIMHIP_TAB_POOL 448
#endif
constexpr int kTabPool = CLSIMHIP_TAB_POOL;
constexpr int kTabSegWords = 12;
constexpr int kTabWaveWords = 2 * kTabPool + 2 * 64 * kTabSegWords;
static_assert(kTabWaveWords >= 2 * kTabSlots + 64 && kTabWaveWords % 4 == 0, "table maker: a wave's LDS region");
constexpr float kEpsilon = 0.00001f;
constexpr float kSpeedOfLight = 0.299792458f;
constexpr float kPi = 3.14159265359f;
constexpr uint32_t kNoStep = 0xffffffffu;
constexpr int kTiltScalarBins = 6;

typedef const __attribute__((address_space(4))) KParams *KP;

DM KP fresh_params(KP p)
{
    asm volatile("" : "+s"(p));
    return p;
}

extern __shared__ __attribute__((aligned(16))) uint32_t lds_words[];

DM uint64_t ballot(bool p) { return __builtin_amdgcn_ballot_w64(p); }

struct Rec4 { float a, b, c, d; };

enum CensusRegion { kCensusCrossing = 0, kCensusFilter = 1, kCensusLiu = 2, kCensusHG = 3, kCensusSearchFull = 4, kCensusSearchNamed = 5,
                    kCensusCreation = 6, kCensusService = 7, kCensusScatter = 8, kCensusWalk = 9, kCensusAim = 10, kCensusRegions = 16 };

DM float lds_log(float x) { return dm::log_with_(x, dm::LdsTable{0u}); }
DM void lds_sincos_2pi(float x, float &s, float &c) { dm::sincos_2pi_with_(x, s, c, dm::LdsTable{4u * dm::kMathLogWords}); }

DM float ldsf(uint32_t i) { return __builtin_bit_cast(float, lds_words[i]); }
DM uint32_t ldsu(uint32_t i) { return lds_words[i]; }
DM Rec4 lds_rec4(uint32_t i) { return *reinterpret_cast<const Rec4 *>(&lds_words[i]); }
DM uint32_t lds_u16(uint32_t off, uint32_t i)
{
    const uint32_t w = lds_words[off + (i >> 1)];
    return (i & 1) ? (w >> 16) : (w & 0xffffu);
}

DM float rng_co(uint64_t &x, uint32_t a)
{
    x = (x & 0xffffffffull) * (uint64_t)a + (x >> 32);
    const uint32_t lo = (uint32_t)x;
    float t;
    asm volatile("s_setreg_imm32_b32 hwreg(HW_REG_MODE, 0, 2), 3\n\t"
                 "v_cvt_f32_u32_e32 %0, %1\n\t"
                 "s_setreg_imm32_b32 hwreg(HW_REG_MODE, 0, 2), 0"
                 : "=v"(t) : "v"(lo));
    return t * 2.3283064365386963e-10f;
}
DM float rng_oc(uint64_t &x, uint32_t a) { return 1.0f - rng_co(x, a); }

DM float sqr(float a) { return a * a; }
DM float div_by(float a, float b, float r, bool ok)
{
    if (ok) {
        const float q = a * r;
        return dm::fma_(dm::fma_(-b, q, a), r, q);
    }
    return a / b;
}
DM float rcp_sel(float x, bool fast) { return fast ? dm::rcp_(x) : 1.0f / x; }
constexpr uint32_t kFastLengths = 32u, kFastMatrices = 64u, kFastAniso = 128u;
template <bool FAST>
DM float div_by_t(float a, float b, float r, bool ok)
{
    if (FAST) { const float q = a * r; return dm::fma_(dm::fma_(-b, q, a), r, q); }
    return div_by(a, b, r, ok);
}
template <bool FAST>
DM float rcp_t(float x, bool fast) { return FAST ? dm::rcp_(x) : rcp_sel(x, fast); }
DM float clampf(float v, float lo, float hi) { v = (v > lo) ? v : lo; return (v < hi) ? v : hi; }
DM int clampi(int v, int lo, int hi) { v = (v > lo) ? v : lo; return (v < hi) ? v : hi; }
DM float clampf_ordered(float v, float lo, float hi) { return __builtin_amdgcn_fmed3f(v, lo, hi); }
DM int clamp_index(int v, int hi)
{
    int r;
    asm("v_med3_i32 %0, %1, 0, %2" : "=v"(r) : "v"(v), "s"(hi));
    return r;
}
DM uint32_t axis_bin_generic_(float t, int nbins)
{
    const float f = __builtin_floorf(t);
    const int b = (f != f) ? 0 : ((f >= 2147483648.0f) ? 2147483647 : ((f < -2147483648.0f) ? (-2147483647 - 1) : (int)f));
    return (uint32_t)(clampi(b, -1, nbins) + 1);
}
DM uint32_t axis_bin_(float t, int nbins)
{
    int b, r;
    asm("v_cvt_flr_i32_f32 %0, %1" : "=v"(b) : "v"(t));
    b = (t != t) ? 0 : b;
    asm("v_med3_i32 %0, %1, -1, %2" : "=v"(r) : "v"(b), "s"(nbins));
    return (uint32_t)(r + 1);
}

struct Vec3 { float x, y, z; };

DM void table_bin_fraction(float start, float step, int n, float wlen, int &bin, float &fraction)
{
    const float q = (wlen - start) / step;
    const float fbin = __builtin_truncf(q);
    fraction = q - fbin;
    bin = (int)fbin;
    if ((bin < 0) || ((bin == 0) && (fraction < 0.0f))) { bin = 0; fraction = 0.0f; }
    else if (bin >= n - 1) { bin = n - 2; fraction = 1.0f; }
}
DM float table_value(uint32_t off, float start, float step, int n, float wlen)
{
    int bin; float fraction;
    table_bin_fraction(start, step, n, wlen, bin, fraction);
    const float a = ldsf(off + (uint32_t)bin), b = ldsf(off + (uint32_t)bin + 1u);
    return a + (b - a) * fraction;
}
DM float phase_ref_index(KP P, float wlen)
{
    if (P->phase_kind == CLSIMHIP_REFINDEX_TABLE) return table_value(P->off_phase, P->phase_start, P->phase_step, P->phase_n, wlen);
    const float x = wlen / P->micrometer;
    return P->n[0] + x * (P->n[1] + x * (P->n[2] + x * (P->n[3] + x * P->n[4])));
}
template <bool FAST = false>
DM float group_velocity(KP P, float wlen)
{
    if (P->group_kind == CLSIMHIP_REFINDEX_TABLE)
        return P->c_light / table_value(P->off_group, P->group_start, P->group_step, P->group_n, wlen);
    const float x = wlen / P->micrometer;
    const float np = P->n[0] + x * (P->n[1] + x * (P->n[2] + x * (P->n[3] + x * P->n[4])));
    if (!FAST && P->group_kind == CLSIMHIP_REFINDEX_DISPERSION) {
        const float n_inv = 1.0f / np;
        const float y = (P->n[1] + x * (2.0f * P->n[2] + x * (3.0f * P->n[3] + x * 4.0f * P->n[4]))) / P->micrometer;
        return P->c_light * (1.0f + y * wlen * n_inv) * n_inv;
    }
    const float np_corr = P->g[0] + x * (P->g[1] + x * (P->g[2] + x * (P->g[3] + x * P->g[4])));
    return P->c_light / (np * np_corr);
}

struct IceFactors { float sca_pow, abs_pow, abs_exp; };

template <int MED>
DM IceFactors ice_factors(KP P, float wlen)
{
    IceFactors f = {0.0f, 0.0f, 0.0f};
    if (MED == CLSIMHIP_LENGTHS_ICECUBE) {
        f.sca_pow = dm::powr_(wlen * P->ref_wlen_recip, P->neg_alpha);
        const float x = wlen / P->nanometer;
        f.abs_pow = dm::powr_(x, P->neg_kappa);
        f.abs_exp = P->abs_A * dm::exp_(P->neg_B / x);
    } else if (MED == CLSIMHIP_LENGTHS_TABLE) {
        int bin;
        table_bin_fraction(P->len_tab_start, P->len_tab_step, P->len_tab_n, wlen, bin, f.sca_pow);
        f.abs_pow = __builtin_bit_cast(float, (uint32_t)(bin * P->num_layers));
    }
    return f;
}
template <int MED, bool FAST = false>
DM void layer_lengths(uint32_t off_layers, const float *len_table, const IceFactors &f, int layer, float &sca_len, float &abs_len,
                      float &rcp_sca, float &rcp_abs, bool fast)
{
    if (MED == CLSIMHIP_LENGTHS_TABLE) {
        const float4 r = *reinterpret_cast<const float4 *>(len_table + 4u * (__builtin_bit_cast(uint32_t, f.abs_pow) + (uint32_t)layer));
        abs_len = r.x + (r.y - r.x) * f.sca_pow;
        sca_len = r.z + (r.w - r.z) * f.sca_pow;
        return;
    }
    const Rec4 r = lds_rec4(off_layers + 4u * (uint32_t)layer);
    if (MED == CLSIMHIP_LENGTHS_ICECUBE) {
        const float x_sca = r.c * f.sca_pow, x_abs = r.a * f.abs_pow + f.abs_exp * r.b;
        sca_len = rcp_t<FAST>(x_sca, fast);
        abs_len = rcp_t<FAST>(x_abs, fast);
        if (FAST || fast) {
            rcp_sca = dm::rcp_of_rcp_(sca_len, x_sca);
            rcp_abs = dm::rcp_of_rcp_(abs_len, x_abs);
        }
    } else {
        sca_len = r.c;
        abs_len = r.a;
    }
}
struct ScatterK {
    float mix_frac, mix_frac_rest, liu_beta, hg_g, hg_one_minus_g2, hg_one_plus_g2, hg_two_g;
    float rcp_mix_frac, rcp_mix_frac_rest, rcp_hg_two_g;
    uint32_t div_ok;
};
static_assert(offsetof(KParams, hg_two_g) - offsetof(KParams, mix_frac) == 24 && offsetof(KParams, liu_beta) - offsetof(KParams, mix_frac) == 8,
              "mix_frac, mix_frac_rest, liu_beta, hg_g, hg_one_minus_g2, hg_one_plus_g2, hg_two_g are seven consecutive floats");
static_assert(offsetof(KParams, div_ok) - offsetof(KParams, rcp_tilt_dz) == 20 && offsetof(KParams, rcp_mix_frac) - offsetof(KParams, rcp_tilt_dz) == 8,
              "rcp_tilt_dz, rcp_layer_thickness, rcp_mix_frac, rcp_mix_frac_rest, rcp_hg_two_g, div_ok are six consecutive words");
static_assert(sizeof(KParams) >= offsetof(KParams, rcp_tilt_dz) + 32 && sizeof(KParams) >= offsetof(KParams, mix_frac) + 32, "the two groups are read as eight words each");
DM ScatterK scatter_constants(KP P)
{
    typedef uint32_t u32x8 __attribute__((ext_vector_type(8)));
    typedef const __attribute__((address_space(4))) u32x8 *group_ptr;
    const u32x8 a = *reinterpret_cast<group_ptr>(&P->mix_frac);
    const u32x8 b = *reinterpret_cast<group_ptr>(&P->rcp_tilt_dz);
    ScatterK K;
    K.mix_frac = dm::u2f(a[0]); K.mix_frac_rest = dm::u2f(a[1]); K.liu_beta = dm::u2f(a[2]); K.hg_g = dm::u2f(a[3]);
    K.hg_one_minus_g2 = dm::u2f(a[4]); K.hg_one_plus_g2 = dm::u2f(a[5]); K.hg_two_g = dm::u2f(a[6]);
    K.rcp_mix_frac = dm::u2f(b[2]); K.rcp_mix_frac_rest = dm::u2f(b[3]); K.rcp_hg_two_g = dm::u2f(b[4]);
    K.div_ok = b[5];
    return K;
}
template <bool FAST = false>
DM float hg_cos(const ScatterK &K, float u)
{
    const float s = 2.0f * u - 1.0f;
    const float ii = FAST ? dm::div_near_(K.hg_one_minus_g2, 1.0f + K.hg_g * s) : K.hg_one_minus_g2 / (1.0f + K.hg_g * s);
    return clampf_ordered(div_by_t<FAST>(K.hg_one_plus_g2 - ii * ii, K.hg_two_g, K.rcp_hg_two_g, FAST || (K.div_ok & 16u) != 0), -1.0f, 1.0f);
}
template <bool FAST = false>
DM float liu_cos(const ScatterK &K, float u)
{
    const float beta = K.liu_beta;
    const float p = (FAST || beta <= 0.09f) ? dm::powr_unit_from_log_(u, beta, lds_log(u)) : dm::powr_(u, beta);
    return clampf_ordered(2.0f * p - 1.0f, -1.0f, 1.0f);
}
template <bool FAST = false>
DM float scattering_cos(KP P, uint64_t &x, uint32_t a)
{
    const ScatterK K = scatter_constants(P);
    const float rr = rng_co(x, a);
    if (!FAST) {
        const int kind = P->scatter_kind;
        if (kind == 0) return hg_cos(K, rr);
        if (kind == 1) return liu_cos(K, rr);
    }
    const uint32_t ok = FAST ? 0xffu : K.div_ok;
    CENSUS_REGION(P, kCensusScatter);
    if (rr < K.mix_frac) {
        CENSUS_REGION(P, kCensusLiu);
        return liu_cos<FAST>(K, div_by_t<FAST>(rr, K.mix_frac, K.rcp_mix_frac, (ok & 4u) != 0));
    }
    CENSUS_REGION(P, kCensusHG);
    return hg_cos<FAST>(K, div_by_t<FAST>(1.0f - rr, K.mix_frac_rest, K.rcp_mix_frac_rest, (ok & 8u) != 0));
}

template <bool FAST = false>
DM float abs_len_corr(KP P, const Vec3 &d)
{
    const float n0 = (P->an_azx * d.x) + (P->an_azy * d.y);
    const float n1 = (P->an_mazy * d.x) + (P->an_azx * d.y);
    const float s0 = n0 * n0, s1 = n1 * n1, s2 = d.z * d.z;
    const float nB = (s0 * P->an_rl[0] + s1 * P->an_rl[1]) + s2 * P->an_rl[2];
    const float An = (s0 * P->an_l[0] + s1 * P->an_l[1]) + s2 * P->an_l[2];
    const float x = (P->an_B2 - nB) * An;
    return (FAST || (P->div_ok & kFastAniso) != 0u) ? 2.0f * dm::rcp_(x) : 2.0f / x;
}
DM void apply_matrix(const __attribute__((address_space(4))) float *m, int renorm, Vec3 &d, bool fast)
{
    const float x = (m[0] * d.x) + (m[1] * d.y) + (m[2] * d.z);
    const float y = (m[3] * d.x) + (m[4] * d.y) + (m[5] * d.z);
    const float z = (m[6] * d.x) + (m[7] * d.y) + (m[8] * d.z);
    d.x = x; d.y = y; d.z = z;
    if (renorm) {
        const float n2 = d.x * d.x + d.y * d.y + d.z * d.z;
        const float norm = fast ? dm::rsqrt_near_(n2) : dm::rsqrt_(n2);
        d.x = d.x * norm; d.y = d.y * norm; d.z = d.z * norm;
    }
}

template <bool FAST = false>
DM float tilt_z_shift(KP P, float px, float py, float pz)
{
    const float z_rescaled = div_by_t<FAST>(pz - P->tilt_first_z, P->tilt_dz, P->rcp_tilt_dz, (P->div_ok & 1u) != 0);
    const int nz = P->tilt_nz, nd = P->tilt_nd;
    const uint32_t off_dist = P->off_tilt_dist;
    const int k = clamp_index((int)__builtin_floorf(z_rescaled), nz - 2);
    const float fraction_z_above = z_rescaled - (float)k;
    const float fraction_z_below = 1.0f - fraction_z_above;
    const float nr = P->tilt_lnx * px + P->tilt_lny * py;
    int j = 1;
    if (FAST || nd <= kTiltScalarBins + 2) {
#pragma unroll
        for (int t = 0; t < kTiltScalarBins; ++t) j += (nr >= P->tilt_inner_dist[t]) ? 1 : 0;
    } else {
        for (int t = 1; t < nd - 1; ++t) j += (nr >= ldsf(off_dist + t)) ? 1 : 0;
    }
    const Rec4 bin = lds_rec4(P->off_tilt_bins + 4u * (uint32_t)j);
    const float thisDist = bin.a;
    const float q = (thisDist - nr) * bin.c;
    float frac_at_lower = dm::fma_(dm::fma_(-bin.b, q, thisDist - nr), bin.c, q);
    if (!FAST && __builtin_bit_cast(uint32_t, bin.d) == 0u) frac_at_lower = (thisDist - nr) / bin.b;
    const float frac_at_upper = 1.0f - frac_at_lower;
    const uint32_t lo = P->off_tilt_zcorr + (uint32_t)((j - 1) * nz + k);
    const uint32_t hi = lo + (uint32_t)nz;
    const float val_at_lower = (ldsf(lo + 1) * fraction_z_above + ldsf(lo) * fraction_z_below);
    const float val_at_upper = (ldsf(hi + 1) * fraction_z_above + ldsf(hi) * fraction_z_below);
    return (val_at_upper * frac_at_upper + val_at_lower * frac_at_lower);
}

DM float generate_wavelength(KP P, int gen, uint64_t &x, uint32_t a)
{
    if (P->gen_kind[gen] == 1) return P->gen_value[gen];
    if (P->gen_kind[gen] == 2) {
        const float u = rng_oc(x, a);
        return 1.0f / (P->gen_first[gen] + u * P->gen_spacing[gen]);
    }
    const float r = rng_oc(x, a);
    const uint32_t cum = P->off_gen_ycum[gen], yv = P->off_gen_yv[gen];
    int lo = 1, hi = P->gen_n[gen] - 1;
    while (lo < hi) {
        const int mid = (lo + hi) >> 1;
        if (ldsf(cum + mid) >= r) hi = mid; else lo = mid + 1;
    }
    const int k = lo - 1;
    const float this_acu = (k == 0) ? 0.0f : ldsf(cum + k);
    const float b = ldsf(yv + k);
    const bool own_x = (P->gen_kind[gen] == 3);
    const float x0 = own_x ? ldsf(P->off_gen_xv[gen] + (uint32_t)k) : (float)k * P->gen_spacing[gen] + P->gen_first[gen];
    const float sp = own_x ? (ldsf(P->off_gen_xv[gen] + (uint32_t)k + 1u) - x0) : P->gen_spacing[gen];
    const float slope = (ldsf(yv + k + 1) - b) / sp;
    const float dy = r - this_acu;
    if ((b == 0.0f) && (slope == 0.0f)) return x0;
    else if (b == 0.0f) return x0 + dm::sqrt_(2.0f * dy / slope);
    else if (slope == 0.0f) return x0 + dy / b;
    else return x0 + (dm::sqrt_(dy * (2.0f * slope) / (b * b) + 1.0f) - 1.0f) * b / slope;
}

DM float wavelength_bias(KP P, float wavelength)
{
    if (P->bias_kind == 1) return P->bias_value;
    const float q = (wavelength - P->bias_start) / P->bias_step;
    const float fbin = __builtin_truncf(q);
    float fraction = q - fbin;
    int ibin = (int)fbin;
    const int n = P->bias_n;
    if ((ibin < 0) || ((ibin == 0) && (fraction < 0.0f))) { ibin = 0; fraction = 0.0f; }
    else if (ibin >= n - 1) { ibin = n - 2; fraction = 1.0f; }
    const uint32_t off = P->off_bias;
    const float v0 = ldsf(off + ibin), v1 = ldsf(off + ibin + 1);
    return v0 + (v1 - v0) * fraction;
// ... 637 lines not shown
```

### clsim_amd/csrc/prop_pool_keep_kernel.hip

```cpp
#include "prop_pool_kernel.hip.h"

namespace clsimhip {

hipError_t launch_pool_keep_kernel(const KParams &P, const KVariant &v, hipStream_t stream)
{
    if (P.n_steps == 0) return hipSuccess;
    if (check_lengths(P, v) != hipSuccess) return hipErrorInvalidValue;
    if (P.history_n != 0 || v.tabulate || !v.keep_detected) return hipErrorInvalidValue;
    if (P.num_layers >= (1 << 14)) return hipErrorInvalidValue;
    if (P.n_steps > kPoolIndexMask) return hipErrorInvalidValue;
    const bool fast = v.fast && !v.generic_only;
    return dispatch_variant(v, fast, [&](auto med, auto tilt, auto aniso, auto flasher, auto fast_tag) {
        return launch_pool_variant<med(), tilt(), aniso(), flasher(), fast_tag(), true>(P, stream, v.grid, v.launched);
    });
}

}
```

### clsim_amd/csrc/prop_pool_kernel.hip

```cpp
#include "prop_pool_kernel.hip.h"

namespace clsimhip {

hipError_t launch_pool_kernel(const KParams &P, const KVariant &v, hipStream_t stream)
{
    if (P.n_steps == 0) return hipSuccess;
    if (check_lengths(P, v) != hipSuccess) return hipErrorInvalidValue;
    if (P.history_n != 0 || v.tabulate || v.keep_detected) return hipErrorInvalidValue;
    if (P.num_layers >= (1 << 14)) return hipErrorInvalidValue;
    if (P.n_steps > kPoolIndexMask) return hipErrorInvalidValue;
    const bool fast = v.fast && !v.generic_only;
    return dispatch_variant(v, fast, [&](auto med, auto tilt, auto aniso, auto flasher, auto fast_tag) {
        return launch_pool_variant<med(), tilt(), aniso(), flasher(), fast_tag(), false>(P, stream, v.grid, v.launched);
    });
}

size_t pool_kernel_max_steps() { return (size_t{1} << kPoolIndexBits) - 1; }
bool pool_kernel_fits(uint32_t table_words, uint32_t keep_strings, int num_layers)
{
    if (num_layers >= (1 << 14)) return false;
    static_assert(kPoolWorthwhileReady >= kPoolMinReady, "an image the pooled kernel is chosen for must be one it can run");
    return pool_ring_that_fits(table_words, keep_strings) >= kPoolWorthwhileReady;
}

}
```

### clsim_amd/csrc/prop_pool_kernel.hip.h

```cpp
#include <hip/hip_runtime.h>

#include <cstdlib>

#include "prop_device.hip.h"
#include "prop_launch.h"

namespace clsimhip {

#define CLSIMHIP_STR2(x) #x
#define CLSIMHIP_STR(x) CLSIMHIP_STR2(x)
#ifndef CLSIMHIP_POOL_BLOCK
#define CLSIMHIP_POOL_BLOCK 768
#define CLSIMHIP_POOL_WAVES 6
#endif
#ifndef CLSIMHIP_POOL_GROUPS
#define CLSIMHIP_POOL_GROUPS 2
#endif
constexpr int kPoolBlock = CLSIMHIP_POOL_BLOCK;
constexpr int kPoolWavesPerBlock = kPoolBlock / 64;
constexpr int kPoolMinWaves = CLSIMHIP_POOL_WAVES;
constexpr uint32_t kReadyWords = 20;
constexpr uint32_t kPendWords = 4;
#ifndef CLSIMHIP_POOL_STAGE
#define CLSIMHIP_POOL_STAGE 4
#endif
constexpr int kPoolStage = CLSIMHIP_POOL_STAGE;
constexpr uint32_t kPoolFixedWords = kPoolStage * kStubWords;
constexpr uint32_t kFlagLast = 1u << 16, kFlagWaiting = 1u << 17;
constexpr int kPoolMinReady = 4;
constexpr int kPoolWorthwhileReady = 8;

__host__ __device__ constexpr uint32_t pool_wave_words(uint32_t R, uint32_t extra) { return (kPoolFixedWords + extra + kReadyWords * R + kPendWords * (64u + R) + 3u) & ~3u; }

constexpr uint32_t kPoolIndexBits = 23, kPoolFlagBits = 18, kPoolIndexMask = (1u << kPoolIndexBits) - 1u;
static_assert(kPoolIndexBits + kPoolFlagBits / 2 == 32 && kPoolFlagBits % 2 == 0, "a pending entry's index (or count) and half of its flags share one word");
static_assert((kFlagWaiting << 1) == (1u << kPoolFlagBits), "slice number + last + waiting are the 18 flag bits");
typedef uint32_t pend_entry __attribute__((ext_vector_type(4)));
DM void pend_store(uint32_t *list, uint32_t k, uint32_t sidx, uint64_t rx, uint32_t left, uint32_t flags)
{
    pend_entry e = {sidx | (flags << 23), (uint32_t)rx, (uint32_t)(rx >> 32), left | ((flags >> 9) << 23)};
    *reinterpret_cast<pend_entry *>(list + kPendWords * k) = e;
}
DM void pend_load(const uint32_t *list, uint32_t k, uint32_t &sidx, uint64_t &rx, uint32_t &left, uint32_t &flags)
{
    const pend_entry e = *reinterpret_cast<const pend_entry *>(list + kPendWords * k);
    sidx = e.x & 0x7fffffu;
    rx = (uint64_t)e.y | ((uint64_t)e.z << 32);
    left = e.w & 0x7fffffu;
    flags = (e.x >> 23) | ((e.w >> 23) << 9);
}
__host__ __device__ constexpr uint32_t pool_keep_extra_words(uint32_t num_strings) { return 64u * ((num_strings + 63u) >> 6); }

template <int MED, bool TILT, bool ANISO, bool FLASHER, bool FAST, bool KEEP>
__global__ void __launch_bounds__(kPoolBlock, kPoolMinWaves) prop_pool_kernel(const KParams Pvalue)
{
    const KP P0 = (KP)__builtin_amdgcn_kernarg_segment_ptr();
    (void)Pvalue;
    {
        const uint32_t words = P0->table_words;
        const uint32_t *src = P0->tables;
        for (uint32_t i = threadIdx.x; i < words; i += kPoolBlock) lds_words[i] = src[i];
    }
    const uint32_t R = (uint32_t)P0->pool_ready;
    const uint32_t U = 64u + R;
    const uint32_t wave_in_group = (uint32_t)__builtin_amdgcn_readfirstlane((int)(threadIdx.x >> 6));
    const uint32_t keep_extra = KEEP ? pool_keep_extra_words((uint32_t)P0->num_strings) : 0u;
    uint32_t *wave_lds = lds_words + ((P0->table_words + 3u) & ~3u) + wave_in_group * pool_wave_words(R, keep_extra);
    uint32_t *stage = wave_lds;
    uint32_t *keep_mask = wave_lds + kPoolFixedWords;
    uint32_t *pend = wave_lds + kPoolFixedWords + keep_extra;
    uint32_t *ready = pend + kPendWords * U;
    __syncthreads();

    const uint32_t lane = threadIdx.x & 63u;
    const uint64_t lanes_below = (1ull << lane) - 1ull;
    const uint32_t n_steps = P0->n_steps;
    uint32_t slice_photons, rounds;
    {
        const uint32_t max_photons = P0->queue[1];
        const uint32_t target = (uint32_t)P0->slices;
        slice_photons = (max_photons + target - 1u) / target;
        if (slice_photons == 0u) slice_photons = 1u;
        if (slice_photons > 0x7fffffu) slice_photons = 0x7fffffu;
        rounds = (max_photons + slice_photons - 1u) / slice_photons;
        if (rounds == 0u) rounds = 1u;
    }
    uint32_t sub_queue = (blockIdx.x * (uint32_t)kPoolWavesPerBlock + wave_in_group) % (uint32_t)kSubQueues;
    uint32_t used_up = 0;
// ... 290 lines not shown
                    bool full = FLASHER ? (ballot(st == kParked) != 0ull) : true;
                    if (!full) {
                        const uint32_t id = st - (kParked + 1u);
                        const uint4 named = fresh_params(P0)->dom_named[id];
                        if (named.x != 0xffffffffu) hit = find_collision_named<FAST>(fresh_params(P0), ph, distance, id, named, hit_string, hit_dom);
                        else full = true;
                    }
                    if (full) hit = find_collision<FAST>(fresh_params(P0), ph, distance, hit_string, hit_dom);
                    st = kLive;
                    advance = true;
                }
                const uint64_t hit_mask = ballot(hit);
                if (__builtin_expect(hit_mask != 0ull, 0)) {
                    const uint32_t total = (uint32_t)__popcll(hit_mask);
                    const uint32_t rank = (uint32_t)__popcll(hit_mask & lanes_below);
                    for (uint32_t done = 0; done < total;) {
                        const uint32_t space = (uint32_t)kPoolStage - n_staged;
                        const uint32_t take = (total - done < space) ? (total - done) : space;
                        if (hit && rank >= done && rank < done + take) {
                            uint32_t *st = stage + (n_staged + rank - done) * kStubWords;
                            st[0] = dm::f2u(ph.px); st[1] = dm::f2u(ph.py); st[2] = dm::f2u(ph.pz); st[3] = dm::f2u(ph.pt);
                            st[4] = dm::f2u(ph.d.x); st[5] = dm::f2u(ph.d.y); st[6] = dm::f2u(ph.d.z); st[7] = dm::f2u(distance);
                            st[8] = dm::f2u(ph.total_path); st[9] = dm::f2u(ph.abs_lens_left); st[10] = dm::f2u(ph.inv_groupvel);
                            st[11] = ph.num_scatters; st[12] = sidx;
                            st[13] = (uint32_t)ph.rx_start; st[14] = (uint32_t)(ph.rx_start >> 32);
                            st[15] = (hit_string & 0xffffu) | (hit_dom << 16);
                        }
                        n_staged += take;
                        done += take;
                        __builtin_amdgcn_fence(__ATOMIC_RELEASE, "wavefront");
                        __builtin_amdgcn_wave_barrier();
                        __builtin_amdgcn_fence(__ATOMIC_ACQUIRE, "wavefront");
                        if (n_staged == (uint32_t)kPoolStage) {
                            flush_hit_stubs(fresh_params(P0), stage, n_staged, lane);
                            n_staged = 0u;
                        }
                    }
                }
            }
        }
        if (advance) {
            if (hit) ph.abs_lens_left = 0.0f;
            ph.px += ph.d.x * distance;
            ph.py += ph.d.y * distance;
            ph.pz += ph.d.z * distance;
            ph.pt += ph.inv_groupvel * distance;
            ph.total_path += distance;
            if (ph.abs_lens_left < kEpsilon) {
                --photons_left;
                st = kSpent;
            } else {
                const KP P = fresh_params(P0);
                if (ANISO && P->has_pre) apply_matrix(P->pre, P->pre_renorm, ph.d, FAST || (P->div_ok & kFastMatrices) != 0u);
                const float cos_s = scattering_cos<FAST>(P, rx, ra);
                const float sin_s = dm::sqrt_near_(1.0f - sqr(cos_s));
                scatter_direction(cos_s, sin_s, ph.d, rng_co(rx, ra));
                if (ANISO && P->has_post) apply_matrix(P->post, P->post_renorm, ph.d, FAST || (P->div_ok & kFastMatrices) != 0u);
                ++ph.num_scatters;
            }
        }
        m_spent = ballot(st == kSpent);
        m_vacant = ballot(st == kVacant);
        m_live = ballot(st >= kLive);
        if (__builtin_expect((m_live | m_spent | (uint64_t)n_left) == 0ull, 0)) break;
    }
    if (n_staged != 0u) flush_hit_stubs(fresh_params(P0), stage, n_staged, lane);
    CENSUS(
    if (lane == 0) {
        unsigned long long *d = fresh_params(P0)->census;
        atomicAdd(d + 0, c_trips); atomicAdd(d + 1, c_run); atomicAdd(d + 2, c_services); atomicAdd(d + 3, c_creations);
        atomicAdd(d + 4, c_created); atomicAdd(d + 5, c_vacant); atomicAdd(d + 6, c_polls); atomicAdd(d + 7, c_parked);
        atomicAdd(d + 9, c_searches); atomicAdd(d + 10, c_chunks); atomicAdd(d + 11, c_empty_ring);
        atomicAdd(d + 12, t_service); atomicAdd(d + 13, t_publish); atomicAdd(d + 14, t_take); atomicAdd(d + 15, t_create);
        atomicAdd(d + 24600, (unsigned long long)__builtin_readcyclecounter() - t_wave_start);
        atomicAdd(d + 24601, t_ring_store); atomicAdd(d + 24602, c_ring_stores); atomicAdd(d + 24603, t_hand_out); atomicAdd(d + 24604, c_hand_outs);
        const uint32_t w = blockIdx.x * (uint32_t)kPoolWavesPerBlock + wave_in_group;
        d[16 + 3 * w] = wall_clock64();
        d[16 + 3 * w + 1] = 0;
        d[16 + 3 * w + 2] = c_trips;
    }
    )
}

static int pool_ring_that_fits(uint32_t table_words, uint32_t keep_strings)
{
    const int budget_words = (160 * 1024 / CLSIMHIP_POOL_GROUPS - 4096 / CLSIMHIP_POOL_GROUPS) / 4 - (int)((table_words + 3u) & ~3u);
    const int per_wave = (budget_words / kPoolWavesPerBlock) & ~3;
    return (per_wave - (int)kPoolFixedWords - (int)pool_keep_extra_words(keep_strings) - (int)kPendWords * 64) / (int)(kReadyWords + kPendWords);
}

template <int MED, bool TILT, bool ANISO, bool FLASHER, bool FAST, bool KEEP>
static hipError_t launch_pool_variant(const KParams &Pin, hipStream_t stream, int grid_wanted = 0, KLaunched *launched = nullptr)
{
    KParams P = Pin;
    if (launched) *launched = KLaunched{KEEP ? CLSIMHIP_FAMILY_POOL_KEEP : CLSIMHIP_FAMILY_POOL, MED, TILT, ANISO, FLASHER, FAST};
    int R = P.pool_ready;
    {
        const int fit = pool_ring_that_fits(P.table_words, KEEP ? (uint32_t)P.num_strings : 0u);
        if (R <= 0 || R > fit) R = fit;
        if (R > 64) R = 64;
        if (R < kPoolMinReady) R = kPoolMinReady;
        if (R > fit) return hipErrorInvalidValue;
        P.pool_ready = R;
    }
    const size_t lds_bytes = (size_t)(((P.table_words + 3u) & ~3u) + kPoolWavesPerBlock * pool_wave_words((uint32_t)R, KEEP ? pool_keep_extra_words((uint32_t)P.num_strings) : 0u)) * 4;
    LaunchPlan plan;
    if (const hipError_t e = plan_launch(reinterpret_cast<const void *>(&prop_pool_kernel<MED, TILT, ANISO, FLASHER, FAST, KEEP>), kPoolBlock, lds_bytes, plan)) return e;
    uint32_t grid = (uint32_t)plan.resident;
    if (P.chip_share > 1) grid = (grid / (uint32_t)P.chip_share > 0u) ? grid / (uint32_t)P.chip_share : 1u;
    if (grid_wanted >= 1 && grid_wanted <= plan.resident) grid = (uint32_t)grid_wanted;
    size_t lds_launch = lds_bytes;
    if (Pin.pool_ready <= 0 && (uint64_t)grid * kPoolWavesPerBlock * (64u + (uint32_t)R) > (uint64_t)P.n_steps) {
        const int smaller = (int)((uint64_t)P.n_steps / ((uint64_t)grid * kPoolWavesPerBlock)) - 64;
        if (smaller >= kPoolWorthwhileReady && smaller < R && 5 * smaller >= 4 * R) {
            R = smaller;
            P.pool_ready = R;
            lds_launch = (size_t)(((P.table_words + 3u) & ~3u) + kPoolWavesPerBlock * pool_wave_words((uint32_t)R, KEEP ? pool_keep_extra_words((uint32_t)P.num_strings) : 0u)) * 4;
        }
    }
    const uint32_t slots_per_group = (uint32_t)kPoolWavesPerBlock * (64u + (uint32_t)R);
    const uint32_t needed = (P.n_steps + slots_per_group - 1u) / slots_per_group;
    if (needed < grid) grid = needed;
    {
        const double r = (double)P.n_steps / ((double)grid * slots_per_group);
        if (P.slices <= 0) P.slices = (r < 0.95) ? 1 : 16;
        if (P.k_search <= 0) P.k_search = (r < 0.95) ? 1 : (FLASHER ? 1 : 5);
        if (P.k_wait < 0) P.k_wait = 16;
        if (P.k_aim < 0) P.k_aim = 8;
        if (P.k_pop <= 0) P.k_pop = 4;
        if (P.k_pop > 64) P.k_pop = 64;
        if (P.k_new <= 0 || P.k_new > R) P.k_new = (R > 8) ? R - 1 : R;
        if (P.k_wait > 255) P.k_wait = 255;
        if (P.k_search > 64) P.k_search = 64;
        if (P.k_aim > 64) P.k_aim = 64;
        P.k_packed = (uint32_t)P.k_pop | ((uint32_t)P.k_search << 8) | ((uint32_t)P.k_aim << 16) | ((uint32_t)P.k_wait << 24);
        if (P.slices > 0xffff) P.slices = 0xffff;
        if ((uint64_t)P.n_steps * (uint64_t)P.slices >= 0x7fffffffull) P.slices = 1;
    }
    hipError_t err = launch_scan_steps(P, stream);
    if (err != hipSuccess) return err;
    hipLaunchKernelGGL((prop_pool_kernel<MED, TILT, ANISO, FLASHER, FAST, KEEP>), dim3(grid), dim3(kPoolBlock), lds_launch, stream, P);
    err = hipGetLastError();
    if (err != hipSuccess) return err;
    return launch_assemble_hits(P, FLASHER, stream);
}

}
```

### include/clsimhip.h

```cpp
#ifndef CLSIMHIP_H
#define CLSIMHIP_H

#include <stddef.h>
#include <stdint.h>

#ifdef __cplusplus
extern "C" {
#endif

#define CLSIMHIP_OK 0
#define CLSIMHIP_ERR_ARGUMENT (-1)
#define CLSIMHIP_ERR_STATE (-2)
#define CLSIMHIP_ERR_CONFIG (-3)
#define CLSIMHIP_ERR_DEVICE (-4)
#define CLSIMHIP_ERR_IO (-5)

typedef struct clsimhip_converter clsimhip_converter;
typedef struct clsimhip_medium clsimhip_medium;

#pragma pack(push, 1)
typedef struct {
    float x, y, z, time;
    float theta, phi, length, beta;
    uint32_t num_photons;
    float weight;
    uint32_t identifier;
    uint8_t source_type, dummy1;
    uint16_t dummy2;
} clsimhip_step;
typedef struct {
    float x, y, z, time;
    float theta, phi, wavelength, cherenkov_dist;
    uint32_t num_scatters;
    float weight;
    uint32_t identifier;
    int16_t string_id;
    uint16_t om_id;
    float start_x, start_y, start_z, start_time;
    float start_theta, start_phi, group_velocity, dist_in_abs_lens;
} clsimhip_photon;
#pragma pack(pop)


#define CLSIMHIP_FUNCTION_TABLE 0
#define CLSIMHIP_FUNCTION_CONSTANT 1
#define CLSIMHIP_FUNCTION_TABLE_X 2
#define CLSIMHIP_FUNCTION_DELTA_PEAK 3
typedef struct {
    int32_t kind;
    int32_t n;
    double start, step;
    const double *values;
    double value;
    const double *wavelengths;
} clsimhip_function;

#define CLSIMHIP_RANDOM_INTERPOLATED 0
#define CLSIMHIP_RANDOM_CONSTANT 1
#define CLSIMHIP_RANDOM_CHERENKOV_NO_DISPERSION 2
#define CLSIMHIP_RANDOM_INTERPOLATED_X 3
typedef struct {
    int32_t kind;
    int32_t n;
    double first, spacing;
    const double *y;
    double value;
    const double *x;
} clsimhip_random_value;

#define CLSIMHIP_LENGTHS_CONSTANT 0
#define CLSIMHIP_LENGTHS_ICECUBE 1
#define CLSIMHIP_LENGTHS_TABLE 2
#define CLSIMHIP_REFINDEX_ICECUBE 0
#define CLSIMHIP_REFINDEX_TABLE 1
#define CLSIMHIP_REFINDEX_DISPERSION 2
#define CLSIMHIP_SCATTER_HG 0
#define CLSIMHIP_SCATTER_LIU 1
#define CLSIMHIP_SCATTER_MIXED 2
typedef struct {
    int32_t num_layers;
    double layers_z_start, layers_height;
    double min_wavelength, max_wavelength;
    int32_t lengths_kind;
    const double *abs_length, *sca_length;
    double alpha, kappa, A, B, D, E;
    const double *a_dust400, *delta_tau, *b400;
    double n[5], g[5];
// ... 43 lines not shown
int clsimhip_get_device(const clsimhip_converter *c, int *out);

int clsimhip_set_wlen_generators(clsimhip_converter *c, const clsimhip_random_value *gens, size_t n);
int clsimhip_set_wlen_bias(clsimhip_converter *c, const clsimhip_function *bias);
int clsimhip_set_medium_properties(clsimhip_converter *c, const clsimhip_medium *m);
int clsimhip_set_geometry(clsimhip_converter *c, size_t n, const int32_t *string_ids, const uint32_t *dom_ids,
                          const double *x, const double *y, const double *z,
                          const char *const *subdetectors, double om_radius);
int clsimhip_set_geometry_from_text_file(clsimhip_converter *c, const char *filename, double om_radius,
                                         int32_t string_id_min, int32_t string_id_max, uint32_t dom_id_min, uint32_t dom_id_max);
int clsimhip_set_enable_double_buffering(clsimhip_converter *c, int value);
int clsimhip_set_double_precision(clsimhip_converter *c, int value);
int clsimhip_set_stop_detected_photons(clsimhip_converter *c, int value);
int clsimhip_set_save_all_photons(clsimhip_converter *c, int value);
int clsimhip_set_save_all_photons_prescale(clsimhip_converter *c, double value);
int clsimhip_set_fixed_number_of_absorption_lengths(clsimhip_converter *c, double value);
int clsimhip_set_dom_pancake_factor(clsimhip_converter *c, double value);
int clsimhip_set_photon_history_entries(clsimhip_converter *c, uint32_t value);
int clsimhip_set_workgroup_size(clsimhip_converter *c, size_t value);
int clsimhip_set_max_num_workitems(clsimhip_converter *c, size_t value);
int clsimhip_compile(clsimhip_converter *c);
int clsimhip_get_max_workgroup_size(const clsimhip_converter *c, size_t *out);
int clsimhip_initialize(clsimhip_converter *c, uint64_t seed);
int clsimhip_initialize_with_streams(clsimhip_converter *c, const uint64_t *x, const uint32_t *a, size_t count);
int clsimhip_is_initialized(const clsimhip_converter *c);

int clsimhip_enqueue_steps(clsimhip_converter *c, const clsimhip_step *steps, size_t n, uint32_t identifier);
int clsimhip_get_conversion_result(clsimhip_converter *c, uint32_t *identifier,
                                   const clsimhip_photon **photons, size_t *n);
int clsimhip_get_result_histories(clsimhip_converter *c, const clsimhip_photon *photons, const float **histories,
                                  uint32_t *entries);
int clsimhip_release_result(clsimhip_converter *c, const clsimhip_photon *photons);
int clsimhip_get_workgroup_size(const clsimhip_converter *c, size_t *out);
int clsimhip_get_max_num_workitems(const clsimhip_converter *c, size_t *out);
int clsimhip_queue_size(const clsimhip_converter *c, size_t *out);
int clsimhip_more_photons_available(const clsimhip_converter *c, int *out);
int clsimhip_get_statistics(const clsimhip_converter *c, double out[8]);
#define CLSIMHIP_OPTION_ENABLE_DOUBLE_BUFFERING 0
#define CLSIMHIP_OPTION_DOUBLE_PRECISION 1
#define CLSIMHIP_OPTION_STOP_DETECTED_PHOTONS 2
#define CLSIMHIP_OPTION_SAVE_ALL_PHOTONS 3
#define CLSIMHIP_OPTION_SAVE_ALL_PHOTONS_PRESCALE 4
#define CLSIMHIP_OPTION_FIXED_NUMBER_OF_ABSORPTION_LENGTHS 5
#define CLSIMHIP_OPTION_DOM_PANCAKE_FACTOR 6
#define CLSIMHIP_OPTION_PHOTON_HISTORY_ENTRIES 7
int clsimhip_get_option(const clsimhip_converter *c, int option, double *out);

int clsimhip_set_tuning(clsimhip_converter *c, const char *key, long long value);
int clsimhip_get_tuning(const clsimhip_converter *c, const char *key, long long *value);

int clsimhip_propagate_device(clsimhip_converter *c, const void *d_steps, size_t n, size_t rng_offset,
                              void *d_photons, size_t capacity, void *d_hit_count, void *stream);
int clsimhip_set_concurrent_device_launches(clsimhip_converter *c, int k);
int clsimhip_replace_indices_with_ids(const clsimhip_converter *c, clsimhip_photon *photons, size_t n);
int clsimhip_kernel_time_ms(clsimhip_converter *c, int reset, double *total_ms, uint64_t *launches);

int clsimhip_step_series_blob_size(size_t n, size_t *bytes);
int clsimhip_encode_step_series(const clsimhip_step *steps, size_t n, uint8_t *out, size_t capacity, size_t *written);
int clsimhip_decode_step_series(const uint8_t *blob, size_t bytes, clsimhip_step *steps_out, size_t capacity, size_t *n, size_t *consumed);
int clsimhip_photon_series_blob_size(size_t n, size_t *bytes);
int clsimhip_encode_photon_series(const clsimhip_photon *photons, size_t n, uint8_t *out, size_t capacity, size_t *written);
int clsimhip_decode_photon_series(const uint8_t *blob, size_t bytes, clsimhip_photon *photons_out, size_t capacity, size_t *n, size_t *consumed);
int clsimhip_encode_portable_uint(uint64_t value, uint8_t out[9], size_t *written);

#define CLSIMHIP_UNIQUE_ID_BYTES 128
typedef struct clsimhip_comm clsimhip_comm;
int clsimhip_comm_get_unique_id(uint8_t id[CLSIMHIP_UNIQUE_ID_BYTES]);
int clsimhip_comm_create(int device_ordinal, int rank, int world_size, const uint8_t id[CLSIMHIP_UNIQUE_ID_BYTES], clsimhip_comm **out);
void clsimhip_comm_destroy(clsimhip_comm *comm);
int clsimhip_comm_info(clsimhip_comm *comm, int *rccl_ranks, int *rccl_rank, int *device_ordinal, char *pci_bus_id, size_t pci_bus_id_bytes);
int clsimhip_comm_statistics(clsimhip_comm *comm, uint64_t *gathers, double *gather_ms, uint64_t *records_sent, uint64_t *records_received, int reset);
int clsimhip_gather_hits(clsimhip_comm *comm, const void *d_photons, const void *d_hit_count, size_t capacity, int root,
                         void *d_gathered, size_t gathered_capacity, uint64_t *counts_out, void *hip_stream);

int clsimhip_kernel_for_bunch(const clsimhip_converter *c, size_t n_steps, int *out);
int clsimhip_uses_pooled_kernel(const clsimhip_converter *c, int *out);
#define CLSIMHIP_FAMILY_CLASSIC 0
#define CLSIMHIP_FAMILY_KEEP 1
#define CLSIMHIP_FAMILY_POOL 2
#define CLSIMHIP_FAMILY_POOL_KEEP 3
#define CLSIMHIP_FAMILY_TAB4 4
#define CLSIMHIP_FAMILY_TAB5 5
int clsimhip_get_last_launch(const clsimhip_converter *c, int out[6]);
long clsimhip_get_table(const clsimhip_converter *c, const char *name, double *out, size_t cap);
int clsimhip_get_rng_state(clsimhip_converter *c, uint64_t *x_out, size_t count);
int clsimhip_eval_math(int device_ordinal, int what, const float *x, const float *y, size_t n, float *out);

#define CLSIMHIP_EVAL_LENGTHS 0
#define CLSIMHIP_EVAL_REFRACTION 1
#define CLSIMHIP_EVAL_WAVELENGTH_BIAS 2
#define CLSIMHIP_EVAL_TILT 3
#define CLSIMHIP_EVAL_ABS_LEN_SCALING 4
#define CLSIMHIP_EVAL_PRE_SCATTER_TRANSFORM 5
#define CLSIMHIP_EVAL_POST_SCATTER_TRANSFORM 6
int clsimhip_eval_device_function(clsimhip_converter *c, int what, int layer, int fast, const float *in4, size_t n, float *out4);
#define CLSIMHIP_EVAL_RANDOM_UNIFORM 0
#define CLSIMHIP_EVAL_RANDOM_WAVELENGTH 1
#define CLSIMHIP_EVAL_RANDOM_SCATTERING_COSINE 2
int clsimhip_eval_device_random(clsimhip_converter *c, int what, int generator, int fast, uint64_t *x, const uint32_t *a, size_t n_streams,
                                size_t draws, float *out);
int clsimhip_check_math_exhaustive(int device_ordinal, int what, int exp_lo, int exp_hi, uint32_t *result, size_t result_cap);

const char *clsimhip_version(void);

#define CLSIMHIP_STEPS_CASCADE 0
#define CLSIMHIP_STEPS_MUON_CASCADE 1
#define CLSIMHIP_STEPS_MUON 2
typedef struct {
    float x, y, z, time;
    float dx, dy, dz;
    float length;
    float pa, pb;
    uint32_t kind;
    uint32_t identifier;
    uint32_t photons_per_step;
    uint32_t num_photons_in_last_step;
    uint64_t num_steps;
} clsimhip_step_request;
int clsimhip_count_generated_steps(const clsimhip_step_request *requests, size_t n, size_t granularity,
                                   size_t *steps_out, size_t *padded_out);
int clsimhip_generate_steps_device(int device, const clsimhip_step_request *requests, size_t n, uint64_t seed,
                                   size_t granularity, void *d_steps, size_t capacity, void *hip_stream, size_t *padded_out);
int clsimhip_generate_steps(int device, const clsimhip_step_request *requests, size_t n, uint64_t seed,
                            size_t granularity, clsimhip_step *steps_out, size_t capacity, size_t *padded_out);

#define CLSIMHIP_PARTICLE_GAMMA 22
#define CLSIMHIP_PARTICLE_EMINUS 11
#define CLSIMHIP_PARTICLE_EPLUS (-11)
#define CLSIMHIP_PARTICLE_MUMINUS 13
#define CLSIMHIP_PARTICLE_MUPLUS (-13)
#define CLSIMHIP_PARTICLE_TAUMINUS 15
#define CLSIMHIP_PARTICLE_TAUPLUS (-15)
#define CLSIMHIP_PARTICLE_PI0 111
#define CLSIMHIP_PARTICLE_PIPLUS 211
#define CLSIMHIP_PARTICLE_PIMINUS (-211)
#define CLSIMHIP_PARTICLE_K0_LONG 130
#define CLSIMHIP_PARTICLE_KPLUS 321
#define CLSIMHIP_PARTICLE_KMINUS (-321)
#define CLSIMHIP_PARTICLE_K0_SHORT 310
#define CLSIMHIP_PARTICLE_PPLUS 2212
#define CLSIMHIP_PARTICLE_PMINUS (-2212)
#define CLSIMHIP_PARTICLE_NEUTRON 2112
#define CLSIMHIP_PARTICLE_BREMS (-2000001001)
#define CLSIMHIP_PARTICLE_DELTAE (-2000001002)
#define CLSIMHIP_PARTICLE_PAIRPROD (-2000001003)
#define CLSIMHIP_PARTICLE_NUCLINT (-2000001004)
#define CLSIMHIP_PARTICLE_HADRONS (-2000001006)
#define CLSIMHIP_SHAPE_OTHER 0
#define CLSIMHIP_SHAPE_CASCADE_SEGMENT 1
typedef struct {
    int32_t type;
    int32_t shape;
    double x, y, z, time;
    double dx, dy, dz;
    double energy;
    double length;
    uint32_t identifier;
    uint32_t reserved;
} clsimhip_particle;
typedef struct {
    uint32_t photons_per_step;
    uint32_t high_photons_per_step;
    double use_high_photons_per_step_from;
    int32_t use_cascade_extension;
    int32_t reserved;
    double medium_density;
// ... 260 lines not shown
```

Before: 4.208 billion.

## JIT-compile pooled propagation kernel with configuration constants baked in via hiprtc

Adds a run-time compiled variant of the pooled propagation kernel. hiprtc generates it from source in which the non-launch KParams members (geometry, scattering and pancake constants) are emitted as compile-time literals. For the IceCube-lengths, tilt, fast, non-aniso, non-flasher configuration it is launched via hipModuleLaunchKernel instead of the AOT kernel. It falls back to the AOT kernel when compilation fails, when the kernel uses more than 80 VGPRs, or when it uses scratch. The goal is to let the compiler constant-fold parameters and cut kernarg/scalar loads, at the price of first-call JIT latency and a dependency on hiprtc.

New measurement: 4.310 billion, median of 6. 2.4% higher.

```diff
diff --git a/clsim_amd/_lib.py b/clsim_amd/_lib.py
--- a/clsim_amd/_lib.py
+++ b/clsim_amd/_lib.py
@@ -2,7 +2,8 @@
 import os
 
 HERE = os.path.dirname(os.path.abspath(__file__))
-LIB_PATH = os.environ.get("CLSIMHIP_LIB", os.path.join(HERE, "libclsimhip.so"))
+DEFAULT_LIB_PATH = os.path.join(HERE, "libclsimhip.so")
+LIB_PATH = os.environ.get("CLSIMHIP_LIB", DEFAULT_LIB_PATH)
 
 OK, ERR_ARGUMENT, ERR_STATE, ERR_CONFIG, ERR_DEVICE, ERR_IO = 0, -1, -2, -3, -4, -5
 REFINDEX_ICECUBE, REFINDEX_TABLE, REFINDEX_DISPERSION = 0, 1, 2
@@ -100,7 +101,7 @@
     "clsimhip_eval_math", "clsimhip_check_math_exhaustive", "clsimhip_version",
     "clsimhip_eval_device_function", "clsimhip_eval_device_random", "clsimhip_get_option",
     "clsimhip_set_tuning", "clsimhip_get_tuning", "clsimhip_tabulator_set_tuning",
-    "clsimhip_get_last_launch", "clsimhip_tabulator_get_last_launch",
+    "clsimhip_get_last_launch", "clsimhip_tabulator_get_last_launch", "clsimhip_baked_info", "clsimhip_baked_compile", "clsimhip_baked_set_compiler_library",
     "clsimhip_count_generated_steps", "clsimhip_generate_steps_device", "clsimhip_generate_steps",
     "clsimhip_ppc_create", "clsimhip_ppc_destroy", "clsimhip_ppc_photons_per_meter", "clsimhip_ppc_enqueue", "clsimhip_shower_parameters",
     "clsimhip_flasher_correction_factor", "clsimhip_flasher_enqueue",
@@ -227,6 +228,9 @@
         "clsimhip_get_tuning": (i32, [vp, C.c_char_p, C.POINTER(C.c_longlong)]),
         "clsimhip_tabulator_set_tuning": (i32, [vp, C.c_char_p, C.c_longlong]),
         "clsimhip_get_last_launch": (i32, [vp, C.POINTER(C.c_int)]),
+        "clsimhip_baked_set_compiler_library": (i32, [C.c_char_p]),
+        "clsimhip_baked_info": (i32, [vp, C.POINTER(C.c_int), C.c_char_p, C.c_char_p, C.c_size_t]),
+        "clsimhip_baked_compile": (i32, [vp, C.c_char_p, C.c_char_p, C.c_char_p, C.c_char_p, C.POINTER(C.c_double), C.c_char_p, C.c_size_t]),
         "clsimhip_tabulator_get_last_launch": (i32, [vp, C.POINTER(C.c_int)]),
         "clsimhip_eval_device_function": (i32, [vp, i32, i32, i32, vp, sz, vp]),
         "clsimhip_eval_device_random": (i32, [vp, i32, i32, i32, vp, vp, sz, sz, vp]),
@@ -304,7 +308,11 @@
         "clsimhip_tabulator_write_fits_file": (i32, [vp, C.c_char_p, C.POINTER(C.c_char_p), C.POINTER(C.c_int32), C.POINTER(C.c_int64), C.POINTER(C.c_double), sz]),
     }
     for name in SYMBOLS:
+        if name in ("clsimhip_baked_info", "clsimhip_baked_compile", "clsimhip_baked_set_compiler_library") and LIB_PATH != DEFAULT_LIB_PATH and not hasattr(lib, name):
+            continue
         fn = getattr(lib, name)
         fn.restype, fn.argtypes = sig[name]
+    if os.environ.get("CLSIMHIP_HIPRTC_LIBRARY") and hasattr(lib, "clsimhip_baked_set_compiler_library"):
+        lib.clsimhip_baked_set_compiler_library(os.fsencode(os.environ["CLSIMHIP_HIPRTC_LIBRARY"]))
     _lib = lib
     return lib
diff --git a/clsim_amd/converter.py b/clsim_amd/converter.py
--- a/clsim_amd/converter.py
+++ b/clsim_amd/converter.py
@@ -756,6 +756,21 @@
         out = (C.c_int * 6)()
         self._call("clsimhip_get_last_launch", out)
         return _lib.launched_dict(out)
+
+    BAKED_STATES = {0: "unused", 1: "baked", 2: "fallback"}
+
+    def GetBakedInfo(self):
+        state, key, why = C.c_int(), C.create_string_buffer(33), C.create_string_buffer(4096)
+        self._call("clsimhip_baked_info", C.byref(state), key, why, len(why))
+        return {"state": self.BAKED_STATES[state.value], "key": key.value.decode(), "why": why.value.decode(errors="replace")}
+
+    def CompileBakedKernel(self, arch="gfx950", flags=None, code_path=None):
+        key, why, seconds = C.create_string_buffer(33), C.create_string_buffer(4096), C.c_double()
+        r = self._lib.clsimhip_baked_compile(self._h, arch.encode(), None if flags is None else flags.encode(),
+                                             None if code_path is None else os.fsencode(code_path), key, C.byref(seconds), why, len(why))
+        if r < 0:
+            _check(int(r), self._h)
+        return {"compiled": bool(r), "key": key.value.decode(), "seconds": seconds.value, "why": why.value.decode(errors="replace")}
 
     EVAL = {"lengths": 0, "refraction": 1, "wavelength_bias": 2, "tilt": 3, "abs_len_scaling": 4, "pre_scatter_transform": 5,
             "post_scatter_transform": 6}
diff --git a/clsim_amd/csrc/baked_kernel.cpp b/clsim_amd/csrc/baked_kernel.cpp
--- /dev/null
+++ b/clsim_amd/csrc/baked_kernel.cpp
@@ -0,0 +1,208 @@
+#include "baked_kernel.h"
+
+#include <dlfcn.h>
+#include <hip/hip_runtime_api.h>
+#include <hip/hip_vector_types.h>
+#include <hip/hiprtc.h>
+
+#include <chrono>
+#include <cstdio>
+#include <cstdlib>
+#include <map>
+#include <mutex>
+#include <sstream>
+#include <utility>
+
+#include "kparams.h"
+
+namespace clsimhip {
+
+namespace {
+
+struct Hiprtc {
+    void *handle = nullptr;
+    std::string error;
+    decltype(&hiprtcVersion) Version = nullptr;
+    decltype(&hiprtcCreateProgram) CreateProgram = nullptr;
+    decltype(&hiprtcCompileProgram) CompileProgram = nullptr;
+    decltype(&hiprtcDestroyProgram) DestroyProgram = nullptr;
+    decltype(&hiprtcGetProgramLog) GetProgramLog = nullptr;
+    decltype(&hiprtcGetProgramLogSize) GetProgramLogSize = nullptr;
+    decltype(&hiprtcGetCode) GetCode = nullptr;
+    decltype(&hiprtcGetCodeSize) GetCodeSize = nullptr;
+};
+
+std::mutex g_library_mutex;
+std::string g_library;
+
+const Hiprtc &hiprtc()
+{
+    static Hiprtc r;
+    static std::once_flag once;
+    std::call_once(once, [] {
+        std::vector<std::string> names;
+        {
+            std::lock_guard<std::mutex> lk(g_library_mutex);
+            if (!g_library.empty()) names.push_back(g_library);
+        }
+        if (names.empty()) names = {"libhiprtc.so.7", "libhiprtc.so", "/opt/rocm/lib/libhiprtc.so"};
+        for (const std::string &n : names) {
+            r.handle = dlopen(n.c_str(), RTLD_NOW | RTLD_LOCAL);
+            if (r.handle) break;
+        }
+        if (!r.handle) {
+            const char *e = dlerror();
+            r.error = std::string("cannot load hiprtc: ") + (e ? e : names.front().c_str());
+            return;
+        }
+        auto sym = [&](const char *name) {
+            void *p = dlsym(r.handle, name);
+            if (!p && r.error.empty()) r.error = std::string("hiprtc symbol missing: ") + name;
+            return p;
+        };
+        r.Version = reinterpret_cast<decltype(r.Version)>(sym("hiprtcVersion"));
+        r.CreateProgram = reinterpret_cast<decltype(r.CreateProgram)>(sym("hiprtcCreateProgram"));
+        r.CompileProgram = reinterpret_cast<decltype(r.CompileProgram)>(sym("hiprtcCompileProgram"));
+        r.DestroyProgram = reinterpret_cast<decltype(r.DestroyProgram)>(sym("hiprtcDestroyProgram"));
+        r.GetProgramLog = reinterpret_cast<decltype(r.GetProgramLog)>(sym("hiprtcGetProgramLog"));
+        r.GetProgramLogSize = reinterpret_cast<decltype(r.GetProgramLogSize)>(sym("hiprtcGetProgramLogSize"));
+        r.GetCode = reinterpret_cast<decltype(r.GetCode)>(sym("hiprtcGetCode"));
+        r.GetCodeSize = reinterpret_cast<decltype(r.GetCodeSize)>(sym("hiprtcGetCodeSize"));
+    });
+    return r;
+}
+
+struct Module {
+    hipModule_t module = nullptr;
+    hipFunction_t function = nullptr;
+    std::string key, why;
+};
+std::mutex g_mutex;
+std::map<std::pair<int, std::string>, Module> g_modules;
+std::map<std::string, std::vector<char>> g_code;
+
+void say_once(const std::string &key, const std::string &why)
+{
+    std::fprintf(stderr, "clsimhip: the pooled kernel of configuration %s runs precompiled (%s)\n", key.empty() ? "(no key)" : key.c_str(), why.c_str());
+}
+
+}
+
+void baked_set_compiler_library(const std::string &path)
+{
+    std::lock_guard<std::mutex> lk(g_library_mutex);
+    g_library = path;
+}
+
+BakedResult baked_compile(const KParams &P, const BakedVariant &v, const char *arch, const char *flags)
+{
+    BakedResult r;
+    const Hiprtc &rtc = hiprtc();
+    if (!rtc.error.empty()) { r.why = rtc.error; return r; }
+    std::string layout;
+    if (!baked_layout_ok(&layout)) { r.why = layout; return r; }
+    int major = 0, minor = 0;
+    if (rtc.Version(&major, &minor) != HIPRTC_SUCCESS) { r.why = "hiprtcVersion failed"; return r; }
+    r.compiler_version = std::to_string(major) + "." + std::to_string(minor);
+    const std::string source = baked_source(P, v);
+    const std::string all_flags = flags ? flags : baked_default_flags();
+    r.key = baked_cache_key(source, all_flags, arch, r.compiler_version);
+    {
+        std::lock_guard<std::mutex> lk(g_mutex);
+        const auto it = g_code.find(r.key);
+        if (it != g_code.end()) { r.code = it->second; r.ok = true; return r; }
+    }
+    std::vector<std::string> words;
+    {
+        std::istringstream in(all_flags);
+        for (std::string w; in >> w;) words.push_back(w);
+        words.push_back(std::string("--offload-arch=") + arch);
+    }
+    std::vector<const char *> options;
+    for (const std::string &w : words) options.push_back(w.c_str());
+    hiprtcProgram prog = nullptr;
+    if (rtc.CreateProgram(&prog, source.c_str(), "prop_pool_kernel_baked.hip", 0, nullptr, nullptr) != HIPRTC_SUCCESS) { r.why = "hiprtcCreateProgram failed"; return r; }
+    const auto t0 = std::chrono::steady_clock::now();
+    const hiprtcResult compiled = rtc.CompileProgram(prog, (int)options.size(), options.data());
+    r.seconds = std::chrono::duration<double>(std::chrono::steady_clock::now() - t0).count();
+    if (compiled != HIPRTC_SUCCESS) {
+        size_t n = 0;
+        std::string log;
+        if (rtc.GetProgramLogSize(prog, &n) == HIPRTC_SUCCESS && n > 1) {
+            log.resize(n);
+            if (rtc.GetProgramLog(prog, &log[0]) != HIPRTC_SUCCESS) log.clear();
+        }
+        r.why = "compile error: " + log.substr(0, 2000);
+    } else {
+        size_t n = 0;
+        if (rtc.GetCodeSize(prog, &n) == HIPRTC_SUCCESS && n != 0) {
+            r.code.resize(n);
+            if (rtc.GetCode(prog, r.code.data()) == HIPRTC_SUCCESS) r.ok = true;
+        }
+        if (!r.ok) { r.code.clear(); r.why = "hiprtcGetCode failed"; }
+    }
+    rtc.DestroyProgram(&prog);
+    if (r.ok) {
+        std::lock_guard<std::mutex> lk(g_mutex);
+        g_code[r.key] = r.code;
+    }
+    return r;
+}
+
+void *baked_pool_function(const KParams &P, const BakedVariant &v, std::string *why, std::string *key_out)
+{
+    int device = 0;
+    if (hipGetDevice(&device) != hipSuccess) { (void)hipGetLastError(); if (why) *why = "no current device"; return nullptr; }
+    const std::pair<int, std::string> id(device, baked_config_bytes(P, v));
+    {
+        std::lock_guard<std::mutex> lk(g_mutex);
+        const auto it = g_modules.find(id);
+        if (it != g_modules.end()) {
+            if (why) *why = it->second.why;
+            if (key_out) *key_out = it->second.key;
+            return it->second.function;
+        }
+    }
+    Module m;
+    hipDeviceProp_t prop;
+    if (hipGetDeviceProperties(&prop, device) != hipSuccess) { (void)hipGetLastError(); m.why = "no device properties"; }
+    else {
+        std::string arch = prop.gcnArchName;
+        arch = arch.substr(0, arch.find(':'));
+        BakedResult r = baked_compile(P, v, arch.c_str(), nullptr);
+        m.key = r.key;
+        if (!r.ok) m.why = r.why;
+        else if (const hipError_t e = hipModuleLoadData(&m.module, r.code.data())) { (void)hipGetLastError(); m.module = nullptr; m.why = std::string("module load: ") + hipGetErrorString(e); }
+        else {
+            hipFunction_t f = nullptr;
+            int regs = 0, scratch = 0;
+            if (const hipError_t e2 = hipModuleGetFunction(&f, m.module, baked_kernel_name(v).c_str())) { (void)hipGetLastError(); m.why = std::string("kernel not in the module: ") + hipGetErrorString(e2); }
+            else if (hipFuncGetAttribute(&regs, HIP_FUNC_ATTRIBUTE_NUM_REGS, f) != hipSuccess || hipFuncGetAttribute(&scratch, HIP_FUNC_ATTRIBUTE_LOCAL_SIZE_BYTES, f) != hipSuccess) {
+                (void)hipGetLastError();
+                m.why = "function attributes unavailable";
+            } else if (regs > 80 || scratch != 0) m.why = "the compiled kernel takes " + std::to_string(regs) + " vector registers and " + std::to_string(scratch) + " bytes of scratch (at most 80 and none)";
+            else m.function = f;
+            if (!m.function) { (void)hipModuleUnload(m.module); m.module = nullptr; }
+        }
+    }
+    std::lock_guard<std::mutex> lk(g_mutex);
+    const auto placed = g_modules.emplace(id, m);
+    if (!placed.second && m.module) (void)hipModuleUnload(m.module);
+    else if (!m.function) say_once(m.key, m.why);
+    if (why) *why = placed.first->second.why;
+    if (key_out) *key_out = placed.first->second.key;
+    return placed.first->second.function;
+}
+
+void baked_disable(const KParams &P, const BakedVariant &v, const std::string &why)
+{
+    int device = 0;
+    if (hipGetDevice(&device) != hipSuccess) { (void)hipGetLastError(); return; }
+    std::lock_guard<std::mutex> lk(g_mutex);
+    Module &m = g_modules[std::make_pair(device, baked_config_bytes(P, v))];
+    if (m.function || m.why.empty()) say_once(m.key, why);
+    m.function = nullptr;
+    m.why = why;
+}
+
+}
diff --git a/clsim_amd/csrc/baked_kernel.h b/clsim_amd/csrc/baked_kernel.h
--- /dev/null
+++ b/clsim_amd/csrc/baked_kernel.h
@@ -0,0 +1,43 @@
+#pragma once
+#include <stddef.h>
+#include <stdint.h>
+
+#include <string>
+#include <vector>
+
+namespace clsimhip {
+
+struct KParams;
+
+struct BakedVariant { int lengths; bool tilt, aniso, flasher, fast, keep; };
+
+enum { kBakedUnused = 0, kBakedActive = 1, kBakedFallback = 2 };
+
+struct BakedReport {
+    int wanted = 0;
+    int state = kBakedUnused;
+    std::string key, why;
+};
+
+bool baked_layout_ok(std::string *why);
+std::string baked_params_struct(const KParams &P);
+std::string baked_source(const KParams &P, const BakedVariant &v);
+std::string baked_kernel_name(const BakedVariant &v);
+const char *baked_default_flags();
+std::string baked_cache_key(const std::string &source, const std::string &flags, const std::string &arch, const std::string &compiler_version);
+std::string baked_config_bytes(const KParams &P, const BakedVariant &v);
+
+struct BakedResult {
+    bool ok = false;
+    std::string why;
+    std::string key;
+    std::string compiler_version;
+    double seconds = 0.0;
+    std::vector<char> code;
+};
+void baked_set_compiler_library(const std::string &path);
+BakedResult baked_compile(const KParams &P, const BakedVariant &v, const char *arch, const char *flags);
+void *baked_pool_function(const KParams &P, const BakedVariant &v, std::string *why, std::string *key_out);
+void baked_disable(const KParams &P, const BakedVariant &v, const std::string &why);
+
+}
diff --git a/clsim_amd/csrc/baked_source.cpp b/clsim_amd/csrc/baked_source.cpp
--- /dev/null
+++ b/clsim_amd/csrc/baked_source.cpp
@@ -0,0 +1,194 @@
+#include "baked_kernel.h"
+
+#include <hip/hip_vector_types.h>
+
+#include <cstdarg>
+#include <cstddef>
+#include <cstdio>
+#include <cstring>
+
+#include "kparams.h"
+
+static const unsigned char kBakedHeaders[] = {
+#include "baked_headers.inc"
+    0};
+
+#ifndef CLSIMHIP_BAKED_FLAGS
+#error "the Makefile passes the run-time compiler's options as CLSIMHIP_BAKED_FLAGS"
+#endif
+
+namespace clsimhip {
+
+namespace {
+
+struct Member {
+    const char *type, *name;
+    size_t offset, size, count;
+    bool launch;
+    char kind;
+};
+template <typename T> constexpr char kind_of();
+template <> constexpr char kind_of<float>() { return 'f'; }
+template <> constexpr char kind_of<int32_t>() { return 'i'; }
+template <> constexpr char kind_of<uint32_t>() { return 'u'; }
+
+#define KP_L(T, N) {#T, #N, offsetof(KParams, N), sizeof(KParams::N), 0, true, 0},
+#define KP_LA(T, N, C) {#T, #N, offsetof(KParams, N), sizeof(KParams::N), (size_t)(C), true, 0},
+#define KP_C(T, N) {#T, #N, offsetof(KParams, N), sizeof(KParams::N), 0, false, kind_of<T>()},
+#define KP_CA(T, N, C) {#T, #N, offsetof(KParams, N), sizeof(KParams::N), (size_t)(C), false, kind_of<T>()},
+const Member kMembers[] = {
+#include "kparams_members.inc"
+};
+#undef KP_L
+#undef KP_LA
+#undef KP_C
+#undef KP_CA
+constexpr size_t kNumMembers = sizeof(kMembers) / sizeof(kMembers[0]);
+
+void append(std::string &s, const char *fmt, ...) __attribute__((format(printf, 2, 3)));
+void append(std::string &s, const char *fmt, ...)
+{
+    char buf[512];
+    va_list ap;
+    va_start(ap, fmt);
+    const int n = vsnprintf(buf, sizeof buf, fmt, ap);
+    va_end(ap);
+    if (n > 0) s.append(buf, (size_t)n < sizeof buf ? (size_t)n : sizeof buf - 1);
+}
+
+void append_value(std::string &s, char kind, uint32_t word)
+{
+    if (kind == 'f') append(s, "__builtin_bit_cast(float, 0x%08xu)", word);
+    else if (kind == 'i') append(s, "(int32_t)0x%08xu", word);
+    else append(s, "0x%08xu", word);
+}
+
+uint64_t fnv1a(uint64_t h, const void *data, size_t n)
+{
+    const unsigned char *p = static_cast<const unsigned char *>(data);
+    for (size_t i = 0; i < n; ++i) { h ^= p[i]; h *= 0x100000001b3ull; }
+    return h;
+}
+
+}
+
+bool baked_layout_ok(std::string *why)
+{
+    size_t cursor = 0;
+    for (size_t i = 0; i < kNumMembers; ++i) {
+        const Member &m = kMembers[i];
+        const size_t align = (m.count ? m.size / m.count : m.size) < 8 ? 4 : 8;
+        const size_t expected = (cursor + align - 1) / align * align;
+        if (m.offset != expected) {
+            if (why) *why = std::string("kparams_members.inc: ") + m.name + " is not where the list puts it";
+            return false;
+        }
+        if (!m.launch && (m.count ? m.size / m.count : m.size) != 4) {
+            if (why) *why = std::string("kparams_members.inc: configuration member ") + m.name + " is not a 32-bit word";
+            return false;
+        }
+        cursor = m.offset + m.size;
+    }
+    if ((cursor + 7) / 8 * 8 != sizeof(KParams)) {
+        if (why) *why = "kparams_members.inc does not reach the end of KParams";
+        return false;
+    }
+    return true;
+}
+
+std::string baked_params_struct(const KParams &P)
+{
+    const unsigned char *bytes = reinterpret_cast<const unsigned char *>(&P);
+    std::string s = "struct KParams { \\\n";
+    size_t cursor = 0;
+    int pads = 0;
+    for (size_t i = 0; i < kNumMembers; ++i) {
+        const Member &m = kMembers[i];
+        if (m.launch) {
+            if (m.offset > cursor) append(s, "    char baked_pad_%d[%zu]; \\\n", pads++, m.offset - cursor);
+            if (m.count) append(s, "    %s %s[%zu]; \\\n", m.type, m.name, m.count);
+            else append(s, "    %s %s; \\\n", m.type, m.name);
+            cursor = m.offset + m.size;
+            continue;
+        }
+        uint32_t w;
+        if (!m.count) {
+            std::memcpy(&w, bytes + m.offset, 4);
+            append(s, "    static constexpr %s %s = ", m.type, m.name);
+            append_value(s, m.kind, w);
+            s += "; \\\n";
+        } else {
+            append(s, "    static constexpr %s %s[%zu] = {", m.type, m.name, m.count);
+            for (size_t k = 0; k < m.count; ++k) {
+                std::memcpy(&w, bytes + m.offset + 4 * k, 4);
+                if (k) s += ", ";
+                append_value(s, m.kind, w);
+            }
+            s += "}; \\\n";
+        }
+    }
+    if (sizeof(KParams) > cursor) append(s, "    char baked_pad_%d[%zu]; \\\n", pads++, sizeof(KParams) - cursor);
+    s += "};\n";
+    return s;
+}
+
+std::string baked_kernel_name(const BakedVariant &v)
+{
+    char buf[128];
+    snprintf(buf, sizeof buf, "_ZN8clsimhip16prop_pool_kernelILi%dELb%dELb%dELb%dELb%dELb%dEEEvNS_7KParamsE", v.lengths, (int)v.tilt, (int)v.aniso,
+             (int)v.flasher, (int)v.fast, (int)v.keep);
+    return buf;
+}
+
+std::string baked_source(const KParams &P, const BakedVariant &v)
+{
+    if (!baked_layout_ok(nullptr)) return std::string();
+    std::string s = "// generated: the pooled propagation kernel of one configuration (baked_source.cpp)\n";
+    s += "typedef signed char int8_t;\ntypedef unsigned char uint8_t;\ntypedef short int16_t;\ntypedef unsigned short uint16_t;\n"
+         "typedef int int32_t;\ntypedef unsigned int uint32_t;\ntypedef long int64_t;\ntypedef unsigned long uint64_t;\ntypedef unsigned long uintptr_t;\n";
+    s += "#define KPARAMS_BAKED_STRUCT \\\n";
+    s += baked_params_struct(P);
+    s += reinterpret_cast<const char *>(kBakedHeaders);
+    s += "\nnamespace clsimhip {\n";
+    append(s, "static_assert(sizeof(KParams) == %zu, \"baked KParams: size\");\n", sizeof(KParams));
+    for (size_t i = 0; i < kNumMembers; ++i) {
+        const Member &m = kMembers[i];
+        if (m.launch) append(s, "static_assert(__builtin_offsetof(KParams, %s) == %zu, \"baked KParams: %s\");\n", m.name, m.offset, m.name);
+    }
+    append(s, "template __global__ void prop_pool_kernel<%d, %s, %s, %s, %s, %s>(const KParams);\n", v.lengths, v.tilt ? "true" : "false",
+           v.aniso ? "true" : "false", v.flasher ? "true" : "false", v.fast ? "true" : "false", v.keep ? "true" : "false");
+    s += "} // namespace clsimhip\n";
+    return s;
+}
+
+const char *baked_default_flags() { return CLSIMHIP_BAKED_FLAGS; }
+
+std::string baked_cache_key(const std::string &source, const std::string &flags, const std::string &arch, const std::string &compiler_version)
+{
+    uint64_t h[2] = {0xcbf29ce484222325ull, 0x84222325cbf29ce4ull};
+    const std::string *parts[] = {&source, &flags, &arch, &compiler_version};
+    for (const std::string *p : parts) {
+        const uint64_t n = p->size();
+        for (uint64_t &x : h) {
+            x = fnv1a(x, p->data(), p->size());
+            x = fnv1a(x, &n, sizeof n);
+        }
+        h[1] = h[1] * 0x9e3779b97f4a7c15ull + 1u;
+    }
+    char buf[40];
+    snprintf(buf, sizeof buf, "%016llx%016llx", (unsigned long long)h[0], (unsigned long long)h[1]);
+    return buf;
+}
+
+std::string baked_config_bytes(const KParams &P, const BakedVariant &v)
+{
+    const char *bytes = reinterpret_cast<const char *>(&P);
+    std::string s;
+    for (size_t i = 0; i < kNumMembers; ++i)
+        if (!kMembers[i].launch) s.append(bytes + kMembers[i].offset, kMembers[i].size);
+    const char tag[6] = {(char)v.lengths, (char)v.tilt, (char)v.aniso, (char)v.flasher, (char)v.fast, (char)v.keep};
+    s.append(tag, sizeof tag);
+    return s;
+}
+
+}
diff --git a/clsim_amd/csrc/baked_source_check.cpp b/clsim_amd/csrc/baked_source_check.cpp
--- /dev/null
+++ b/clsim_amd/csrc/baked_source_check.cpp
@@ -0,0 +1,82 @@
+#include <hip/hip_vector_types.h>
+
+#include <cstdio>
+#include <cstring>
+#include <string>
+
+#include "baked_kernel.h"
+#include "kparams.h"
+
+using namespace clsimhip;
+
+static int failures = 0;
+#define CHECK(cond) do { if (!(cond)) { std::fprintf(stderr, "%s:%d: %s\n", __FILE__, __LINE__, #cond); ++failures; } } while (0)
+
+int main()
+{
+    std::string why;
+    CHECK(baked_layout_ok(&why));
+    if (!why.empty()) std::fprintf(stderr, "%s\n", why.c_str());
+
+    KParams P;
+    std::memset(&P, 0, sizeof P);
+    P.num_layers = 171;
+    P.layer_thickness = 10.0f;
+    P.prox_n = 512;
+    P.tilt_dz = -0.0f;
+    P.post_renorm = -1;
+    for (int i = 0; i < 9; ++i) P.pre[i] = 0.125f * (float)i;
+    for (int i = 0; i < kMaxGenerators; ++i) P.off_gen_yv[i] = 0xfffffff0u + (uint32_t)i;
+    P.tables = reinterpret_cast<const uint32_t *>(0x1234);
+    P.n_steps = 77;
+    const BakedVariant v{1, true, false, false, true, false};
+
+    const std::string body = baked_params_struct(P);
+    CHECK(body.find("static constexpr int32_t num_layers = (int32_t)0x000000abu;") != std::string::npos);
+    CHECK(body.find("static constexpr float layer_thickness = __builtin_bit_cast(float, 0x41200000u);") != std::string::npos);
+    CHECK(body.find("static constexpr float tilt_dz = __builtin_bit_cast(float, 0x80000000u);") != std::string::npos);
+    CHECK(body.find("static constexpr int32_t post_renorm = (int32_t)0xffffffffu;") != std::string::npos);
+    CHECK(body.find("static constexpr float pre[9] = {__builtin_bit_cast(float, 0x00000000u), __builtin_bit_cast(float, 0x3e000000u)") != std::string::npos);
+    CHECK(body.find("0xfffffff7u}") != std::string::npos);
+    CHECK(body.find("const uint32_t * tables;") != std::string::npos);
+    CHECK(body.find("uint32_t n_steps;") != std::string::npos);
+    CHECK(body.find("static constexpr uint32_t n_steps") == std::string::npos);
+    CHECK(body.find("1234") == std::string::npos);
+    for (size_t at = 0, end; (end = body.find('\n', at)) != std::string::npos; at = end + 1)
+        CHECK(end + 1 == body.size() || (end > 0 && body[end - 1] == '\\'));
+
+    const std::string source = baked_source(P, v);
+    CHECK(!source.empty());
+    CHECK(source.find("static_assert(sizeof(KParams) == " + std::to_string(sizeof(KParams))) != std::string::npos);
+    CHECK(source.find("static_assert(__builtin_offsetof(KParams, k_packed) == " + std::to_string(offsetof(KParams, k_packed))) != std::string::npos);
+    CHECK(source.find("template __global__ void prop_pool_kernel<1, true, false, false, true, false>(const KParams);") != std::string::npos);
+    CHECK(source.find("__launch_bounds__(kPoolBlock, kPoolMinWaves) prop_pool_kernel") != std::string::npos);
+    CHECK(source.find("#include") == std::string::npos);
+    CHECK(baked_kernel_name(v) == "_ZN8clsimhip16prop_pool_kernelILi1ELb1ELb0ELb0ELb1ELb0EEEvNS_7KParamsE");
+
+    const std::string flags = baked_default_flags();
+    CHECK(flags.find("-ffp-contract=off") != std::string::npos && flags.find("-amdgpu-sdwa-peephole=0") != std::string::npos);
+    const std::string key = baked_cache_key(source, flags, "gfx950", "7.2");
+    CHECK(key.size() == 32);
+    KParams Q = P;
+    Q.tables = nullptr;
+    Q.n_steps = 78;
+    Q.k_packed = 5;
+    CHECK(baked_cache_key(baked_source(Q, v), flags, "gfx950", "7.2") == key);
+    CHECK(baked_config_bytes(Q, v) == baked_config_bytes(P, v));
+    Q.hg_g = 0.5f;
+    CHECK(baked_cache_key(baked_source(Q, v), flags, "gfx950", "7.2") != key);
+    CHECK(baked_config_bytes(Q, v) != baked_config_bytes(P, v));
+    BakedVariant w = v;
+    w.keep = true;
+    CHECK(baked_cache_key(baked_source(P, w), flags, "gfx950", "7.2") != key);
+    CHECK(baked_config_bytes(P, w) != baked_config_bytes(P, v));
+    CHECK(baked_cache_key(source, flags + " -DX", "gfx950", "7.2") != key);
+    CHECK(baked_cache_key(source, flags, "gfx942", "7.2") != key);
+    CHECK(baked_cache_key(source, flags, "gfx950", "7.3") != key);
+    CHECK(baked_cache_key(source + "gfx", flags, "950", "7.2") != baked_cache_key(source, flags, "gfx950", "7.2"));
+
+    if (failures) return 1;
+    std::printf("baked source check ok: %zu bytes of source, key %s\n", source.size(), key.c_str());
+    return 0;
+}
diff --git a/clsim_amd/csrc/c_api.cpp b/clsim_amd/csrc/c_api.cpp
--- a/clsim_amd/csrc/c_api.cpp
+++ b/clsim_amd/csrc/c_api.cpp
@@ -410,6 +410,39 @@
 {
     return guarded_const(c, [&] { need(c, "converter"); need(out, "out"); *out = c->impl.pooled_for(n_steps) ? 1 : 0; });
 }
+int clsimhip_baked_compile(const clsimhip_converter *c, const char *arch, const char *flags, const char *code_path, char key[33], double *seconds,
+                           char *why, size_t why_bytes)
+{
+    int compiled = 0;
+    const int status = guarded_const(c, [&] {
+        need(c, "converter"); need(arch, "arch");
+        const BakedResult r = c->impl.baked_compile_probe(arch, flags);
+        if (key) std::snprintf(key, 33, "%s", r.key.c_str());
+        if (seconds) *seconds = r.seconds;
+        if (why && why_bytes) std::snprintf(why, why_bytes, "%s", r.why.c_str());
+        if (r.ok && code_path) {
+            std::FILE *f = std::fopen(code_path, "wb");
+            if (!f || std::fwrite(r.code.data(), 1, r.code.size(), f) != r.code.size()) { if (f) std::fclose(f); throw Error(CLSIMHIP_ERR_ARGUMENT, "cannot write the code object"); }
+            std::fclose(f);
+        }
+        compiled = r.ok ? 1 : 0;
+    });
+    return status != CLSIMHIP_OK ? status : compiled;
+}
+int clsimhip_baked_set_compiler_library(const char *path)
+{
+    return guarded(nullptr, [&] { baked_set_compiler_library(path ? path : ""); });
+}
+int clsimhip_baked_info(const clsimhip_converter *c, int *state, char key[33], char *why, size_t why_bytes)
+{
+    return guarded_const(c, [&] {
+        need(c, "converter");
+        const BakedReport r = c->impl.baked_report();
+        if (state) *state = r.state;
+        if (key) std::snprintf(key, 33, "%s", r.key.c_str());
+        if (why && why_bytes) std::snprintf(why, why_bytes, "%s", r.why.c_str());
+    });
+}
 int clsimhip_get_device(const clsimhip_converter *c, int *out)
 {
     return guarded_const(c, [&] { need(c, "converter"); need(out, "out"); *out = c->impl.device(); });
diff --git a/clsim_amd/csrc/converter.cpp b/clsim_amd/csrc/converter.cpp
--- a/clsim_amd/csrc/converter.cpp
+++ b/clsim_amd/csrc/converter.cpp
@@ -26,11 +26,16 @@
     v.generic_only = tuning.generic_only;
     KLaunched launched;
     v.launched = &launched;
+    BakedReport baked;
+    if (pooled && tuning.baked_kernel == 2) baked.wanted = 2;
+    else if (pooled && tuning.baked_kernel == 1 && P.n_steps * static_cast<size_t>(concurrent_launches_) >= kPooledKernelMinSteps) baked.wanted = 1;
+    v.baked = &baked;
     const hipError_t err = v.keep_detected ? (pooled ? launch_pool_keep_kernel(P, v, stream) : launch_keep_kernel(P, v, stream))
                                            : (pooled ? launch_pool_kernel(P, v, stream) : launch_prop_kernel(P, v, stream));
     if (launched.family >= 0) {
         std::lock_guard<std::mutex> lk(launched_mutex_);
         launched_ = launched;
+        if (baked.state != kBakedUnused) baked_ = baked;
     }
     return err;
 }
@@ -75,6 +80,7 @@
     {"k_aim", -1, 64, LAUNCH_FIELD(k_aim)},
     {"grid", 0, 1 << 20, LAUNCH_FIELD(grid)},
     {"generic_kernels", 0, 1, LAUNCH_FIELD(generic_only)},
+    {"baked_kernel", 0, 2, LAUNCH_FIELD(baked_kernel)},
     {"result_min_records", 1, 1ll << 32, LAUNCH_FIELD(result_min_records)},
     {"string_map_cells", 8, 4096, TABLE_FIELD(string_map_cells)},
     {"dom_map_cells", 4, 512, TABLE_FIELD(dom_map_cells)},
@@ -103,9 +109,23 @@
 
 long long Converter::get_tuning(const std::string &key) const
 {
+    if (key == "baked_state") return baked_report().state;
     const TuningKey &k = tuning_key(key);
     std::lock_guard<std::mutex> lk(tuning_mutex_);
     return k.get(tuning_, table_tuning_);
+}
+
+BakedResult Converter::baked_compile_probe(const char *arch, const char *flags) const
+{
+    BakedResult r;
+    if (!compiled_) { r.why = "Compile() first"; return r; }
+    const KVariant &v = tables_.variant;
+    LaunchTuning t;
+    {
+        std::lock_guard<std::mutex> lk(tuning_mutex_);
+        t = tuning_;
+    }
+    return baked_compile(tables_.params, BakedVariant{v.lengths, v.tilt, v.aniso, v.flasher, v.fast && !t.generic_only, v.keep_detected}, arch, flags);
 }
 
 void Converter::set_concurrent_device_launches(int k)
diff --git a/clsim_amd/csrc/converter.h b/clsim_amd/csrc/converter.h
--- a/clsim_amd/csrc/converter.h
+++ b/clsim_amd/csrc/converter.h
@@ -12,6 +12,7 @@
 
 #include "hip_resources.h"
 #include "host_model.h"
+#include "baked_kernel.h"
 #include "kparams.h"
 #include "prop_launch.h"
 
@@ -215,6 +216,7 @@
     int k_wait = -1, k_aim = -1;
     int grid = 0;
     bool generic_only = false;
+    int baked_kernel = 1;
     size_t result_min_records = 65536;
     bool derived = false;
     bool use_pool = false;
@@ -293,6 +295,8 @@
     int concurrent_device_launches() const { return concurrent_launches_; }
     bool uses_pooled_kernel() const { need_init(); const LaunchTuning t = tuning_snapshot(); return t.use_pool && t.pool_min_steps == 0; }
     KLaunched last_launch() const { std::lock_guard<std::mutex> lk(launched_mutex_); return launched_; }
+    BakedReport baked_report() const { std::lock_guard<std::mutex> lk(launched_mutex_); return baked_; }
+    BakedResult baked_compile_probe(const char *arch, const char *flags) const;
 
 private:
     using StepPool = PinnedPool<clsimhip_step>;
@@ -453,6 +457,7 @@
     hipError_t launch(const KParams &P, const LaunchTuning &tuning, hipStream_t stream) const;
     mutable std::mutex launched_mutex_;
     mutable KLaunched launched_;
+    mutable BakedReport baked_;
 
     std::unique_ptr<BoundedQueue<Job>> in_queue_;
     std::unique_ptr<BoundedQueue<Result>> out_queue_;
diff --git a/clsim_amd/csrc/detmath.hip.h b/clsim_amd/csrc/detmath.hip.h
--- a/clsim_amd/csrc/detmath.hip.h
+++ b/clsim_amd/csrc/detmath.hip.h
@@ -1,6 +1,8 @@
 #pragma once
+#ifndef __HIPCC_RTC__
 #include <hip/hip_runtime.h>
 #include <stdint.h>
+#endif
 
 #include "math_tables.h"
 
diff --git a/clsim_amd/csrc/embed_headers.py b/clsim_amd/csrc/embed_headers.py
--- /dev/null
+++ b/clsim_amd/csrc/embed_headers.py
@@ -0,0 +1,15 @@
+#!/usr/bin/env python3
+import sys
+
+
+def main():
+    source, target = sys.argv[1], sys.argv[2]
+    with open(source, "rb") as f:
+        data = f.read()
+    with open(target, "w") as f:
+        for i in range(0, len(data), 32):
+            f.write(",".join(str(b) for b in data[i:i + 32]) + ",\n")
+
+
+if __name__ == "__main__":
+    main()
diff --git a/clsim_amd/csrc/kparams.h b/clsim_amd/csrc/kparams.h
--- a/clsim_amd/csrc/kparams.h
+++ b/clsim_amd/csrc/kparams.h
@@ -1,5 +1,7 @@
 #pragma once
+#ifndef __HIPCC_RTC__
 #include <stdint.h>
+#endif
 
 namespace clsimhip {
 
@@ -33,6 +35,9 @@
 static_assert(sizeof(DevStep) == 48, "step record");
 static_assert(sizeof(DevPhoton) == 80, "photon record");
 
+#ifdef KPARAMS_BAKED
+KPARAMS_BAKED
+#else
 struct KParams {
     const uint32_t *tables;
     uint32_t table_words;
@@ -144,10 +149,13 @@
     float dom_mul_x, dom_mul_y;
     uint32_t k_packed;
 };
+#endif
 
 struct KLaunched {
     int family = -1, lengths = -1, tilt = -1, aniso = -1, flasher = -1, fast = -1;
 };
+
+struct BakedReport;
 
 struct KVariant {
     int lengths;
@@ -161,6 +169,7 @@
     bool generic_only = false;
     bool tab_fast = false;
     KLaunched *launched = nullptr;
+    BakedReport *baked = nullptr;
 };
 
 }
diff --git a/clsim_amd/csrc/kparams_members.inc b/clsim_amd/csrc/kparams_members.inc
--- /dev/null
+++ b/clsim_amd/csrc/kparams_members.inc
@@ -0,0 +1,184 @@
+KP_L(const uint32_t *, tables)
+KP_L(uint32_t, table_words)
+KP_L(const DevStep *, steps)
+KP_L(uint32_t, n_steps)
+KP_L(uint64_t *, rng_x)
+KP_L(const uint32_t *, rng_a)
+KP_L(DevPhoton *, out)
+KP_L(uint32_t *, hit_count)
+KP_L(uint32_t, max_hits)
+KP_L(uint32_t *, queue)
+KP_L(int32_t, k_new)
+KP_L(int32_t, k_search)
+KP_L(int32_t, k_wait)
+KP_L(int32_t, k_aim)
+KP_L(int32_t, slices)
+KP_L(int32_t, pool_ready)
+KP_L(int32_t, k_pop)
+KP_L(int32_t, chip_share)
+#ifdef CLSIMHIP_CENSUS
+KP_L(unsigned long long *, census)
+#endif
+KP_L(WorkRecord *, work)
+KP_L(const float *, len_table)
+KP_L(float *, hist_ring)
+KP_L(float *, hist_out)
+KP_C(int32_t, history_n)
+KP_C(int32_t, has_fixed_abs)
+KP_C(float, fixed_abs)
+KP_L(const uint32_t *, prox_map)
+KP_C(int32_t, prox_n)
+KP_C(float, prox_x0)
+KP_C(float, prox_y0)
+KP_C(float, prox_inv_cell)
+KP_C(float, prox_reach)
+KP_L(const uint4 *, dom_cells)
+KP_L(const float4 *, dom_centres)
+KP_L(const uint4 *, dom_named)
+KP_L(const int16_t *, id_strings)
+KP_L(const uint16_t *, id_doms)
+KP_L(const uint32_t *, id_dom_start)
+KP_C(int32_t, dprox_nx)
+KP_C(int32_t, dprox_ny)
+KP_C(int32_t, dprox_nz)
+KP_C(float, dprox_x0)
+KP_C(float, dprox_y0)
+KP_C(float, dprox_z0)
+KP_C(float, dprox_inv_cell)
+KP_C(float, dprox_radius)
+KP_L(const int16_t *, dom_tx)
+KP_L(const int16_t *, dom_ty)
+KP_L(const float *, dom_tz)
+KP_C(int32_t, dom_in_lds)
+KP_C(uint32_t, off_dom_xy)
+KP_C(uint32_t, off_dom_z)
+KP_C(int32_t, num_layers)
+KP_C(float, layer_bottom)
+KP_C(float, layer_thickness)
+KP_C(float, recip_thickness)
+KP_C(uint32_t, off_layers)
+KP_C(float, neg_kappa)
+KP_C(float, abs_A)
+KP_C(float, neg_B)
+KP_C(float, neg_alpha)
+KP_C(float, ref_wlen_recip)
+KP_C(float, nanometer)
+KP_CA(float, n, 5)
+KP_CA(float, g, 5)
+KP_C(float, micrometer)
+KP_C(float, c_light)
+KP_C(int32_t, len_tab_n)
+KP_C(float, len_tab_start)
+KP_C(float, len_tab_step)
+KP_C(int32_t, phase_kind)
+KP_C(int32_t, group_kind)
+KP_C(int32_t, phase_n)
+KP_C(int32_t, group_n)
+KP_C(float, phase_start)
+KP_C(float, phase_step)
+KP_C(float, group_start)
+KP_C(float, group_step)
+KP_C(uint32_t, off_phase)
+KP_C(uint32_t, off_group)
+KP_C(float, mix_frac)
+KP_C(float, mix_frac_rest)
+KP_C(float, liu_beta)
+KP_C(float, hg_g)
+KP_C(float, hg_one_minus_g2)
+KP_C(float, hg_one_plus_g2)
+KP_C(float, hg_two_g)
+KP_CA(float, an_l, 3)
+KP_CA(float, an_rl, 3)
+KP_C(float, an_azx)
+KP_C(float, an_azy)
+KP_C(float, an_mazy)
+KP_C(float, an_B2)
+KP_C(float, abs_corr_const)
+KP_CA(float, pre, 9)
+KP_CA(float, post, 9)
+KP_C(int32_t, has_abs_corr)
+KP_C(int32_t, has_pre)
+KP_C(int32_t, has_post)
+KP_C(int32_t, pre_renorm)
+KP_C(int32_t, post_renorm)
+KP_C(int32_t, scatter_kind)
+KP_C(float, tilt_const)
+KP_C(int32_t, tilt_nd)
+KP_C(int32_t, tilt_nz)
+KP_C(float, tilt_first_z)
+KP_C(float, tilt_dz)
+KP_C(float, tilt_lnx)
+KP_C(float, tilt_lny)
+KP_C(uint32_t, off_tilt_dist)
+KP_C(uint32_t, off_tilt_zcorr)
+KP_C(uint32_t, off_tilt_bins)
+KP_CA(float, tilt_inner_dist, 6)
+KP_C(float, rcp_tilt_dz)
+KP_C(float, rcp_layer_thickness)
+KP_C(float, rcp_mix_frac)
+KP_C(float, rcp_mix_frac_rest)
+KP_C(float, rcp_hg_two_g)
+KP_C(uint32_t, div_ok)
+KP_C(int32_t, num_gen)
+KP_CA(int32_t, gen_kind, kMaxGenerators)
+KP_CA(int32_t, gen_n, kMaxGenerators)
+KP_CA(float, gen_first, kMaxGenerators)
+KP_CA(float, gen_spacing, kMaxGenerators)
+KP_CA(float, gen_value, kMaxGenerators)
+KP_CA(uint32_t, off_gen_yv, kMaxGenerators)
+KP_CA(uint32_t, off_gen_ycum, kMaxGenerators)
+KP_CA(uint32_t, off_gen_xv, kMaxGenerators)
+KP_C(int32_t, bias_kind)
+KP_C(int32_t, bias_n)
+KP_C(float, bias_start)
+KP_C(float, bias_step)
+KP_C(float, bias_value)
+KP_C(uint32_t, off_bias)
+KP_L(double *, tab_bins)
+KP_L(double *, tab_sq_bins)
+KP_LA(float, tab_ref, 12)
+KP_L(uint32_t, off_tab)
+KP_L(int32_t, tab_axes_kind)
+KP_L(int32_t, tab_full_azimuth)
+KP_L(int32_t, tab_ndim)
+KP_LA(float, tab_scale, 5)
+KP_LA(float, tab_offset, 5)
+KP_LA(int32_t, tab_inverse, 5)
+KP_LA(int32_t, tab_nbins, 5)
+KP_LA(float, tab_inv_exp, 5)
+KP_LA(uint32_t, tab_stride, 5)
+KP_L(uint32_t, tab_tiled)
+KP_LA(uint32_t, tab_tile_stride, 3)
+KP_LA(uint32_t, tab_tile_bits, 3)
+KP_L(uint32_t, tab_std)
+KP_L(float, tab_max0)
+KP_L(float, tab_max3)
+KP_L(float, tab_min_inv_groupvel)
+KP_L(float, tab_tan_thetac)
+KP_L(float, tab_volume_step)
+KP_L(int32_t, ang_n)
+KP_L(uint32_t, off_ang)
+KP_L(int32_t, ang_has_min)
+KP_L(int32_t, ang_has_max)
+KP_L(float, ang_min)
+KP_L(float, ang_max)
+KP_L(float, ang_underflow)
+KP_L(float, ang_overflow)
+KP_C(int32_t, has_pancake)
+KP_C(float, pancake)
+KP_C(float, unpancake)
+KP_C(float, om_radius)
+KP_C(float, om_radius_sq)
+KP_C(float, string_max_radius_sq)
+KP_C(float, string_max_radius)
+KP_C(int32_t, num_strings)
+KP_C(int32_t, num_sets)
+KP_C(int32_t, max_layers)
+KP_C(int32_t, num_subdet)
+KP_C(uint32_t, off_strings)
+KP_C(uint32_t, off_sets)
+KP_C(uint32_t, off_layer_to_om)
+KP_C(uint32_t, off_subdet)
+KP_C(float, dom_mul_x)
+KP_C(float, dom_mul_y)
+KP_L(uint32_t, k_packed)
diff --git a/clsim_amd/csrc/prop_device.hip.h b/clsim_amd/csrc/prop_device.hip.h
--- a/clsim_amd/csrc/prop_device.hip.h
+++ b/clsim_amd/csrc/prop_device.hip.h
@@ -1,5 +1,7 @@
 #pragma once
+#ifndef __HIPCC_RTC__
 #include <hip/hip_runtime.h>
+#endif
 
 #include "detmath.hip.h"
 #include "../../include/clsimhip.h"
@@ -101,6 +103,9 @@
 DM float clampf_ordered(float v, float lo, float hi) { return __builtin_amdgcn_fmed3f(v, lo, hi); }
 DM int clamp_index(int v, int hi)
 {
+#ifdef KPARAMS_BAKED
+    if (__builtin_constant_p(hi)) return clampi(v, 0, hi);
+#endif
     int r;
     asm("v_med3_i32 %0, %1, 0, %2" : "=v"(r) : "v"(v), "s"(hi));
     return r;
@@ -207,6 +212,17 @@
     float rcp_mix_frac, rcp_mix_frac_rest, rcp_hg_two_g;
     uint32_t div_ok;
 };
+#ifdef KPARAMS_BAKED
+DM ScatterK scatter_constants(KP P)
+{
+    ScatterK K;
+    K.mix_frac = P->mix_frac; K.mix_frac_rest = P->mix_frac_rest; K.liu_beta = P->liu_beta; K.hg_g = P->hg_g;
+    K.hg_one_minus_g2 = P->hg_one_minus_g2; K.hg_one_plus_g2 = P->hg_one_plus_g2; K.hg_two_g = P->hg_two_g;
+    K.rcp_mix_frac = P->rcp_mix_frac; K.rcp_mix_frac_rest = P->rcp_mix_frac_rest; K.rcp_hg_two_g = P->rcp_hg_two_g;
+    K.div_ok = P->div_ok;
+    return K;
+}
+#else
 static_assert(offsetof(KParams, hg_two_g) - offsetof(KParams, mix_frac) == 24 && offsetof(KParams, liu_beta) - offsetof(KParams, mix_frac) == 8,
               "mix_frac, mix_frac_rest, liu_beta, hg_g, hg_one_minus_g2, hg_one_plus_g2, hg_two_g are seven consecutive floats");
 static_assert(offsetof(KParams, div_ok) - offsetof(KParams, rcp_tilt_dz) == 20 && offsetof(KParams, rcp_mix_frac) - offsetof(KParams, rcp_tilt_dz) == 8,
@@ -225,6 +241,7 @@
     K.div_ok = b[5];
     return K;
 }
+#endif
 template <bool FAST = false>
 DM float hg_cos(const ScatterK &K, float u)
 {
@@ -270,7 +287,8 @@
     const float x = (P->an_B2 - nB) * An;
     return (FAST || (P->div_ok & kFastAniso) != 0u) ? 2.0f * dm::rcp_(x) : 2.0f / x;
 }
-DM void apply_matrix(const __attribute__((address_space(4))) float *m, int renorm, Vec3 &d, bool fast)
+template <typename M>
+DM void apply_matrix(M m, int renorm, Vec3 &d, bool fast)
 {
     const float x = (m[0] * d.x) + (m[1] * d.y) + (m[2] * d.z);
     const float y = (m[3] * d.x) + (m[4] * d.y) + (m[5] * d.z);
diff --git a/clsim_amd/csrc/prop_pool_keep_kernel.hip b/clsim_amd/csrc/prop_pool_keep_kernel.hip
--- a/clsim_amd/csrc/prop_pool_keep_kernel.hip
+++ b/clsim_amd/csrc/prop_pool_keep_kernel.hip
@@ -11,7 +11,7 @@
     if (P.n_steps > kPoolIndexMask) return hipErrorInvalidValue;
     const bool fast = v.fast && !v.generic_only;
     return dispatch_variant(v, fast, [&](auto med, auto tilt, auto aniso, auto flasher, auto fast_tag) {
-        return launch_pool_variant<med(), tilt(), aniso(), flasher(), fast_tag(), true>(P, stream, v.grid, v.launched);
+        return launch_pool_variant<med(), tilt(), aniso(), flasher(), fast_tag(), true>(P, stream, v.grid, v.launched, v.baked);
     });
 }
 
diff --git a/clsim_amd/csrc/prop_pool_kernel.hip b/clsim_amd/csrc/prop_pool_kernel.hip
--- a/clsim_amd/csrc/prop_pool_kernel.hip
+++ b/clsim_amd/csrc/prop_pool_kernel.hip
@@ -11,7 +11,7 @@
     if (P.n_steps > kPoolIndexMask) return hipErrorInvalidValue;
     const bool fast = v.fast && !v.generic_only;
     return dispatch_variant(v, fast, [&](auto med, auto tilt, auto aniso, auto flasher, auto fast_tag) {
-        return launch_pool_variant<med(), tilt(), aniso(), flasher(), fast_tag(), false>(P, stream, v.grid, v.launched);
+        return launch_pool_variant<med(), tilt(), aniso(), flasher(), fast_tag(), false>(P, stream, v.grid, v.launched, v.baked);
     });
 }
 
diff --git a/clsim_amd/csrc/prop_pool_kernel.hip.h b/clsim_amd/csrc/prop_pool_kernel.hip.h
--- a/clsim_amd/csrc/prop_pool_kernel.hip.h
+++ b/clsim_amd/csrc/prop_pool_kernel.hip.h
@@ -1,9 +1,14 @@
+#ifndef __HIPCC_RTC__
 #include <hip/hip_runtime.h>
 
 #include <cstdlib>
+#endif
 
 #include "prop_device.hip.h"
+#ifndef __HIPCC_RTC__
+#include "baked_kernel.h"
 #include "prop_launch.h"
+#endif
 
 namespace clsimhip {
 
@@ -460,6 +465,7 @@
     )
 }
 
+#ifndef __HIPCC_RTC__
 static int pool_ring_that_fits(uint32_t table_words, uint32_t keep_strings)
 {
     const int budget_words = (160 * 1024 / CLSIMHIP_POOL_GROUPS - 4096 / CLSIMHIP_POOL_GROUPS) / 4 - (int)((table_words + 3u) & ~3u);
@@ -468,7 +474,7 @@
 }
 
 template <int MED, bool TILT, bool ANISO, bool FLASHER, bool FAST, bool KEEP>
-static hipError_t launch_pool_variant(const KParams &Pin, hipStream_t stream, int grid_wanted = 0, KLaunched *launched = nullptr)
+static hipError_t launch_pool_variant(const KParams &Pin, hipStream_t stream, int grid_wanted = 0, KLaunched *launched = nullptr, BakedReport *baked = nullptr)
 {
     KParams P = Pin;
     if (launched) *launched = KLaunched{KEEP ? CLSIMHIP_FAMILY_POOL_KEEP : CLSIMHIP_FAMILY_POOL, MED, TILT, ANISO, FLASHER, FAST};
@@ -517,10 +523,30 @@
     }
     hipError_t err = launch_scan_steps(P, stream);
     if (err != hipSuccess) return err;
-    hipLaunchKernelGGL((prop_pool_kernel<MED, TILT, ANISO, FLASHER, FAST, KEEP>), dim3(grid), dim3(kPoolBlock), lds_launch, stream, P);
+    constexpr bool kBakedPays = (MED == CLSIMHIP_LENGTHS_ICECUBE) && TILT && !ANISO && !FLASHER && FAST;
+    bool baked_launched = false;
+    if (baked && (baked->wanted == 2 || (baked->wanted == 1 && kBakedPays))) {
+        const BakedVariant bv{MED, TILT, ANISO, FLASHER, FAST, KEEP};
+        std::string why;
+        if (void *function = baked_pool_function(P, bv, &why, &baked->key)) {
+            size_t bytes = sizeof(P);
+            void *config[] = {HIP_LAUNCH_PARAM_BUFFER_POINTER, &P, HIP_LAUNCH_PARAM_BUFFER_SIZE, &bytes, HIP_LAUNCH_PARAM_END};
+            const hipError_t e = hipModuleLaunchKernel(static_cast<hipFunction_t>(function), grid, 1, 1, kPoolBlock, 1, 1, (unsigned int)lds_launch, stream, nullptr, config);
+            if (e == hipSuccess) baked_launched = true;
+            else {
+                (void)hipGetLastError();
+                why = std::string("launch: ") + hipGetErrorString(e);
+                baked_disable(P, bv, why);
+            }
+        }
+        baked->state = baked_launched ? kBakedActive : kBakedFallback;
+        baked->why = why;
+    }
+    if (!baked_launched) hipLaunchKernelGGL((prop_pool_kernel<MED, TILT, ANISO, FLASHER, FAST, KEEP>), dim3(grid), dim3(kPoolBlock), lds_launch, stream, P);
     err = hipGetLastError();
     if (err != hipSuccess) return err;
     return launch_assemble_hits(P, FLASHER, stream);
 }
+#endif
 
 }
diff --git a/include/clsimhip.h b/include/clsimhip.h
--- a/include/clsimhip.h
+++ b/include/clsimhip.h
@@ -1,8 +1,10 @@
 #ifndef CLSIMHIP_H
 #define CLSIMHIP_H
 
+#ifndef __HIPCC_RTC__
 #include <stddef.h>
 #include <stdint.h>
+#endif
 
 #ifdef __cplusplus
 extern "C" {
@@ -212,6 +214,10 @@
 #define CLSIMHIP_FAMILY_TAB4 4
 #define CLSIMHIP_FAMILY_TAB5 5
 int clsimhip_get_last_launch(const clsimhip_converter *c, int out[6]);
+int clsimhip_baked_set_compiler_library(const char *path);
+int clsimhip_baked_info(const clsimhip_converter *c, int *state, char key[33], char *why, size_t why_bytes);
+int clsimhip_baked_compile(const clsimhip_converter *c, const char *arch, const char *flags, const char *code_path, char key[33], double *seconds,
+                           char *why, size_t why_bytes);
 long clsimhip_get_table(const clsimhip_converter *c, const char *name, double *out, size_t cap);
 int clsimhip_get_rng_state(clsimhip_converter *c, uint64_t *x_out, size_t count);
 int clsimhip_eval_math(int device_ordinal, int what, const float *x, const float *y, size_t n, float *out);
```
